# twndus/YelpRecommendation

Hardware: AMD Instinct MI355X
Metric: BPR triplets/sec @ dim64 (higher is better)
Workload: dtype f32; 1 GPU; BPR-MF dim=64 train step (gather+score+loss+grad+dense Adam), synthetic Yelp2018 shape; users=31668, items=38048, interactions=1566260, train_triplets_per_epoch=920629, batch_per_gpu=524288, global_batch=524288, optimizer=adam(dense), parallelism=single

## Files before the change

include/yelprec_engine.h:

```cpp
#ifndef YELPREC_ENGINE_H
#define YELPREC_ENGINE_H

#include <stdint.h>

#ifdef __cplusplus
extern "C" {
#endif

#define YR_ENGINE_VERSION 36

#define YR_ERR_UNSUPPORTED (-1)
#define YR_ERR_BADARG      (-2)

#define YR_FLAG_BAD_USER 1
#define YR_FLAG_BAD_ITEM 2

#define YR_PULL_USER_PHASE 1
#define YR_PULL_ITEM_PHASE 2

#define YR_S3REC_TRAIN 0
#define YR_S3REC_VALID 1
#define YR_S3REC_TEST  2

#define YR_OPT_ADAM  0
#define YR_OPT_ADAMW 1

#define YR_LOSS_PARTIALS 2048
#define YR_COUNT_SLOTS 64
#define YR_COUNT_WORDS 2048

int yr_engine_version(void);

const char *yr_engine_arch(void);

int yr_mf_score(const float *U, const float *I,
                const int64_t *user, const int64_t *item,
                int64_t B, int D, int64_t num_users, int64_t num_items,
                float *out, int32_t *err_flag, void *stream);

int yr_mf_score_backward(const float *U, const float *I,
                         const int64_t *user, const int64_t *item, const float *gout,
                         int64_t B, int D, int64_t num_users, int64_t num_items,
                         float *gradU, float *gradI, int32_t *err_flag, void *stream);

int yr_bpr_mf_fwd_bwd(const float *U, const float *I,
                      const int64_t *user, const int64_t *pos, const int64_t *neg,
                      int64_t B, int D, int64_t num_users, int64_t num_items,
                      float inv_batch, float *gradU, float *gradI,
                      float *loss_partials, int32_t *err_flag, void *stream);

int yr_bpr_mf_scatter_step(float *U, float *I, float *gradU, float *gradI,
                           float *mU, float *vU, float *mI, float *vI, uint8_t *touched,
                           const int64_t *user, const int64_t *pos, const int64_t *neg,
                           int64_t B, int D, int64_t num_users, int64_t num_items, float inv_batch,
                           double lr, double step_size, double bc2_sqrt,
                           double beta1, double beta2, double eps, double weight_decay, int mode,
                           float *loss_partials, float *loss_out, double *loss_accum,
                           int32_t *err_flag, void *stream);
int yr_adam_dense_dual(float *p0, float *g0, float *m0, float *v0, int64_t n0,
                       float *p1, float *g1, float *m1, float *v1, int64_t n1,
                       int row_width, uint8_t *touched0, uint8_t *touched1,
                       double lr, double step_size, double bc2_sqrt,
                       double beta1, double beta2, double eps, double weight_decay, int mode,
                       const float *loss_partials, float loss_scale, float *loss_out, double *loss_accum,
                       void *stream);

int64_t yr_bpr_mf_pull_workspace_bytes(int64_t max_batch, int64_t num_users, int64_t num_items, int D);
int yr_bpr_mf_pull_step(const float *U_old, float *U_new, float *I,
                        float *mU, float *vU, float *mI, float *vI, float *gradI_out,
                        const int64_t *user, const int64_t *pos, const int64_t *neg,
                        int64_t B, int D, int64_t num_users, int64_t num_items, float inv_batch,
                        double lr, double step_size, double bc2_sqrt,
                        double beta1, double beta2, double eps, double weight_decay, int mode,
                        int deterministic, void *workspace, int64_t workspace_bytes,
                        float *loss_partials, float *loss_out, double *loss_accum,
                        int32_t *err_flag, void *stream);

int yr_bpr_mf_pull_index(const int64_t *user, const int64_t *pos, const int64_t *neg, int64_t B, int D,
                         int64_t num_users, int64_t num_items,
                         void *workspace, int64_t workspace_bytes, int32_t *err_flag, void *stream);
int yr_bpr_mf_pull_apply(const float *U_old, float *U_new, float *I,
                         float *mU, float *vU, float *mI, float *vI, float *gradI_out,
                         int64_t B, int D, int64_t num_users, int64_t num_items, float inv_batch,
                         double lr, double step_size, double bc2_sqrt,
                         double beta1, double beta2, double eps, double weight_decay, int mode,
                         int deterministic, void *workspace, int64_t workspace_bytes,
                         float *loss_partials, float *loss_out, double *loss_accum,
                         int phases, int64_t item_row_begin, int64_t item_row_end,
                         void *stream);
int yr_bpr_mf_pull_item_buckets(int64_t num_items, int D);
int yr_bpr_mf_pull_split_summary(const void *workspace, int64_t workspace_bytes, int64_t B, int D,
                                 int64_t num_users, int64_t num_items, int32_t *counters_out,
                                 int32_t *parts_out, int32_t *rule_out, void *stream);
int yr_bpr_mf_pull_apply_ordered(const float *U_old, float *U_new, float *I,
                         float *mU, float *vU, float *mI, float *vI, float *gradI_out,
                         int64_t B, int D, int64_t num_users, int64_t num_items, float inv_batch,
                         double lr, double step_size, double bc2_sqrt,
                         double beta1, double beta2, double eps, double weight_decay, int mode,
                         int deterministic, void *workspace, int64_t workspace_bytes,
                         float *loss_partials, float *loss_out, double *loss_accum,
                         int phases, int64_t item_row_begin, int64_t item_row_end,
                         const int32_t *item_bucket_order, void *stream);

#define YR_NGCF_MAX_LAYERS 8
int yr_ngcf_score_fwd(const float *const *layers, int n_layers, const int64_t *user, const int64_t *pos,
                      const int64_t *neg, int64_t B, int D, int64_t num_users, int64_t num_items,
                      float *out_pos, float *out_neg, int32_t *err_flag, void *stream);
int yr_ngcf_score_bwd(const float *const *layers, float *const *dlayers, int n_layers, const int64_t *user,
                      const int64_t *pos, const int64_t *neg, const float *gpos, const float *gneg,
                      int64_t B, int D, int64_t num_users, int64_t num_items, int32_t *err_flag, void *stream);
int yr_spmm_csr(const int32_t *rowptr, const int32_t *col, const float *val,
                const float *X, float *Y, int64_t n, int D, int accumulate,
                const int32_t *heavy_rows, int64_t n_heavy, int heavy_threshold, void *stream);
int yr_spmm_csr_sliced(const int32_t *rowptr, const int32_t *col, const float *val,
                       const float *X, float *Y, int64_t n, int D, int accumulate,
                       const int32_t *row_order, void *stream);
int yr_ngcf_dense_fwd(const float *E, const float *Z, const float *W1, const float *W2,
                      int64_t n, int D, float *Eout, void *stream);
int yr_ngcf_dense_bwd_data(const float *dEout, const float *Eout, const float *E, const float *Z,
                           const float *W1T, const float *W2T, int64_t n, int D,
                           float *dZ, float *dE, void *stream);
int yr_ngcf_dense_bwd_weight(const float *dEout, const float *Eout, const float *E, const float *Z,
                             int64_t n, int D, float *dW1, float *dW2, void *stream);

int yr_ngcf_frontier_mark(const int64_t *user, const int64_t *pos, const int64_t *neg, int64_t B,
                          int64_t num_users, int64_t num_items,
                          int32_t *flags, int32_t *rows, int32_t *count, int clear, void *stream);
int yr_ngcf_frontier_expand(const int32_t *rowptr, const int32_t *col, int64_t n,
                            const int32_t *rows_in, const int32_t *count_in, int64_t max_rows_in,
                            int32_t *flags, int32_t *rows, int32_t *count, int clear, void *stream);
int yr_spmm_csr_subset(const int32_t *rowptr, const int32_t *col, const float *val,
                       const float *X, float *Y, int64_t n, int D, int accumulate,
                       const int32_t *heavy_rows, int64_t n_heavy, int heavy_threshold,
                       const int32_t *row_active,
                       const int32_t *row_list, const int32_t *row_count, int64_t max_rows, void *stream);
int yr_spmm_csr_push_rows(const int32_t *rowptr, const int32_t *col, const float *val,
                          const float *X, float *Y, int64_t n, int D,
                          const int32_t *rows, const int32_t *count, int64_t max_rows, void *stream);
int yr_ngcf_dense_fwd_rows(const float *E, const float *Z, const float *W1, const float *W2,
                           int64_t n, int D, float *Eout,
                           const int32_t *rows, const int32_t *count, int64_t max_rows, float *zero_rows,
                           void *stream);
int yr_ngcf_dense_bwd_data_rows(const float *dEout, const float *Eout, const float *E, const float *Z,
                                const float *W1T, const float *W2T, int64_t n, int D, float *dZ, float *dE,
                                const int32_t *rows, const int32_t *count, int64_t max_rows, void *stream);
int yr_ngcf_dense_bwd_weight_rows(const float *dEout, const float *Eout, const float *E, const float *Z,
                                  int64_t n, int D, float *dW1, float *dW2,
                                  const int32_t *rows, const int32_t *count, int64_t max_rows, void *stream);

int64_t yr_ngcf_step_workspace_bytes(int64_t n, int D, int K, int64_t B);
int yr_ngcf_bpr_step(const int32_t *rowptr, const int32_t *col, const float *val, int64_t n, int64_t nnz,
                     const int32_t *heavy_rows, int64_t n_heavy, int heavy_threshold, int64_t num_users,
                     float *const *params, float *const *exp_avg, float *const *exp_avg_sq, int K, int D,
                     const int64_t *user, const int64_t *pos, const int64_t *neg, int64_t B,
                     double lr, double step_size, double bc2_sqrt, double beta1, double beta2, double eps,
                     double weight_decay, int mode, double subset_fraction,
                     void *workspace, int64_t workspace_bytes, float *loss_out, double *loss_accum,
                     int32_t *err_flag, void *stream);

int yr_gemm_f32(int transA, int transB, int64_t M, int64_t N, int64_t K,
                const float *A, int64_t lda, const float *B, int64_t ldb, float *C, int64_t ldc,
                const float *bias, int act, int accumulate, int split_k, void *stream);
int yr_gemm_f32_ex(int transA, int transB, int64_t M, int64_t N, int64_t K,
                   const float *A, int64_t lda, const float *B, int64_t ldb, float *C, int64_t ldc,
                   const float *bias, int act, int accumulate, int split_k,
                   const int32_t *alpha_count, float *rowsum, void *stream);
int64_t yr_cdae_decode_loss_partials(int64_t B, int64_t I);
int yr_cdae_decode_loss(const float *z, const float *Wo, const float *bo, const float *target,
                        const float *negative_mask, int64_t B, int64_t I, int H, int act, float *G,
                        int64_t ldg, float *pred, float *partial_loss, int32_t *count, void *stream);
int yr_cdae_hidden_bwd(float *dz, const float *z, int act, const int64_t *user, int64_t B, int H,
                       int64_t num_users, float *dV, uint8_t *touched_users, float *dbh,
                       const float *partial_loss, int64_t n_partials, const int32_t *count,
                       float *stats, double *loss_accum, int scale_dz, void *stream);
int yr_cdae_compact_pair(const float *x, const float *negative_mask, int64_t B, int64_t I, uint64_t seed,
                         double p, int32_t *cols, float *vals, int32_t *count, int32_t *loss_cols,
                         float *loss_targets, int32_t *loss_count, void *stream);
int yr_cdae_train_lists(const int64_t *ptr, const int64_t *idx, const int64_t *ptr2, const int64_t *idx2,
                        const int64_t *users, int64_t B,
                        int64_t num_users, int64_t I, int neg_times, uint64_t neg_seed,
                        uint64_t drop_seed, double p, int32_t *cols, float *vals, int32_t *count,
                        int32_t *loss_cols, float *loss_targets, int32_t *loss_count,
                        int32_t *err_flag, void *stream);
int yr_cdae_train_lists_batched(const int64_t *ptr, const int64_t *idx, const int64_t *ptr2, const int64_t *idx2,
                                const int64_t *users, int64_t B, int64_t num_users, int64_t I, int neg_times,
                                const uint64_t *neg_seeds, const uint64_t *drop_seeds, int64_t batch_rows, double p,
                                int32_t *cols, float *vals, int32_t *count, int32_t *loss_cols, float *loss_targets,
                                int32_t *loss_count, int32_t *err_flag, void *stream);
int yr_cdae_loss_finalize_batched(const float *partial_loss, int splits, const int32_t *loss_count, int64_t rows,
                                  int64_t batch_rows, float *means, int32_t *arrive, double *loss_accum,
                                  void *stream);
int yr_cdae_sampled_decode_splits(int64_t B);
int yr_cdae_loss_finalize(const float *partial_loss, int64_t n_partials, const int32_t *count, float *stats,
                          double *loss_accum, void *stream);
int yr_cdae_sampled_decode(const int32_t *loss_cols, const float *loss_targets, const int32_t *loss_count,
                           const float *z, const float *Wo, const float *bo, int64_t B, int64_t I, int H,
                           int act, float *dz, float *dWo, float *dbo, float *partial_loss,
                           int32_t *count, void *stream);
int yr_cdae_hidden_init(float *zpre, const float *bias, const float *V, const int64_t *user,
                        int64_t B, int H, int64_t num_users, int32_t *err_flag, void *stream);
int yr_dropout(const float *x, const float *rnd, double p, int64_t n, float *out, void *stream);
int yr_sigmoid(float *x, int64_t n, void *stream);
int yr_dropout_seeded(const float *x, uint64_t seed, double p, int64_t n, float *out, void *stream);
int yr_sigmoid_bwd(const float *dy, const float *y, float *g, int64_t n, void *stream);
int yr_colsum(const float *X, int64_t rows, int64_t cols, float *out, int accumulate, void *stream);
int yr_row_scatter_add(const float *G, const int64_t *user, int64_t B, int H, int64_t num_users,
                       float *dV, void *stream);
int yr_nsbce_fwd(const float *pred, const float *target, const float *negative_mask, int64_t n,
                 float *workspace, float *stats, void *stream);
int yr_nsbce_bwd(const float *pred, const float *target, const float *negative_mask,
                 const float *stats, const float *gout, int64_t n, float *dpred, void *stream);

int yr_loss_finalize(const float *loss_partials, float scale,
                     float *loss_out, double *loss_accum, void *stream);

int yr_mf_scores_gemm(const float *U, const float *I, const int64_t *users, int64_t nrows, int D,
                      int64_t num_users, int64_t num_items, float *scores, int64_t row_stride,
                      int32_t *err_flag, void *stream);

#define YR_EVAL_F32 0
#define YR_EVAL_BF16X3 1
#define YR_EVAL_NO_PRESCAN 2
#define YR_EVAL_FORCE_PRESCAN 4
#define YR_EVAL_TWO_ROLES 8
#define YR_EVAL_FOUR_WAVES 16
int64_t yr_mf_eval_topk_planes_bytes(int64_t num_items, int D);
int64_t yr_mf_eval_topk_workspace_bytes(int64_t nrows, int64_t num_items, int D, int k, int mode);
int yr_mf_eval_topk(const float *U, const float *I, const int64_t *users, int64_t nrows, int D,
                    int64_t num_users, int64_t num_items,
                    const int64_t *mask_ptr, const int64_t *mask_idx, float mask_value,
                    int k, int64_t *out, void *workspace, int64_t workspace_bytes, int mode,
                    const int64_t *hint, int32_t *err_flag, void *stream);
int yr_mf_eval_topk_bias(const float *U, const float *I, const float *item_bias, const int64_t *users,
                         int64_t nrows, int D, int64_t num_users, int64_t num_items,
                         const int64_t *mask_ptr, const int64_t *mask_idx, float mask_value,
                         int k, int64_t *out, void *workspace, int64_t workspace_bytes, int mode,
                         const int64_t *hint, int32_t *err_flag, void *stream);
int64_t yr_ngcf_eval_topk_workspace_bytes(int64_t nrows, int64_t num_items, int n_layers, int D, int k);
int yr_ngcf_eval_topk(const float *const *layers, int n_layers, int D, const int64_t *users, int64_t nrows,
                      int64_t num_users, int64_t num_items,
                      const int64_t *mask_ptr, const int64_t *mask_idx, float mask_value,
                      int k, int64_t *out, void *workspace, int64_t workspace_bytes,
                      const int64_t *hint, int32_t *err_flag, void *stream);

int yr_topk_masked(const float *scores, int64_t nrows, int64_t ncols, int64_t row_stride,
                   const int64_t *mask_ptr, const int64_t *mask_idx, const int64_t *mask_rows,
                   float mask_value, int k, int64_t *out, void *stream);

int64_t yr_rank_metrics_workspace_bytes(int64_t n);
int yr_rank_metrics(const int64_t *topk, int64_t n, int k, const int64_t *pos_ptr, const int64_t *pos_idx,
                    const int64_t *pos_rows, double *workspace, double *out, void *stream);

int yr_bpr_loss_fwd(const float *pos, const float *neg, int64_t B,
                    float *loss_partials, void *stream);
int yr_bpr_loss_bwd(const float *pos, const float *neg, const float *gout,
                    float inv_batch, int64_t B, float *gpos, float *gneg, void *stream);

int yr_adam_dense(float *p, float *g, float *m, float *v, int64_t n,
                  double lr, double step_size, double bc2_sqrt,
                  double beta1, double beta2, double eps, double weight_decay,
                  int mode, int zero_grad, void *stream);

#define YR_ADAM_MULTI_MAX 16
int yr_adam_dense_flat(float *const *p, float *const *g, float *const *m, float *const *v,
                       const int64_t *n, uint8_t *const *touched, const int *row_width, const int *clear,
                       const int *scaled, const int32_t *grad_count, int count, double lr, double step_size, double bc2_sqrt, double beta1,
                       double beta2, double eps, double weight_decay, int mode, void *stream);
int yr_sgd_dense(float *p, float *g, int64_t n, double lr, double weight_decay,
                 int zero_grad, void *stream);

int yr_csr_rows_to_dense(const int64_t *ptr, const int64_t *idx, const int64_t *users, int64_t B,
                         int64_t num_users, int64_t num_items, int accumulate, float *out,
                         int32_t *err_flag, void *stream);
int yr_negative_mask(const float *positives, int64_t B, int64_t num_items, int neg_times, uint64_t seed,
                     float *out, int32_t *err_flag, void *stream);

int64_t yr_cdae_sparse_part_columns(int64_t I);
int yr_cdae_compact_rows(const float *x, int64_t B, int64_t I, uint64_t seed, double p,
                         int32_t *cols, float *vals, int32_t *count, void *stream);
int yr_cdae_sparse_encode(const int32_t *cols, const float *vals, const int32_t *count,
                          const float *Wh, const float *bh, const float *V, const int64_t *user,
                          int64_t B, int64_t I, int H, int64_t num_users, int act, float *z,
                          int32_t *err_flag, void *stream);
int yr_cdae_sparse_dwh(const int32_t *cols, const float *vals, const int32_t *count,
                       const float *dz, int64_t B, int64_t I, int H, float *dWh,
                       float *scratch_T, int32_t *claim, int32_t epoch, int32_t *touched, int32_t *n_touched,
                       void *stream);
int yr_cdae_sparse_encode_t(const int32_t *cols, const float *vals, const int32_t *count, const float *WhT,
                            const float *bh, const float *V, const int64_t *user, int64_t B, int64_t I,
                            int H, int64_t num_users, int act, float *z, int32_t *err_flag, void *stream);
int yr_cdae_sparse_dwh_t(const int32_t *cols, const float *vals, const int32_t *count, const float *dz,
                         int64_t B, int64_t I, int H, float *dWhT, uint8_t *touched_items, void *stream);
int yr_cdae_hidden_bwd_dwh_t(const int32_t *cols, const float *vals, const int32_t *count, const float *dz,
                             const float *z, int act, int scale_dz, const int32_t *pos_count,
                             const int64_t *user, int64_t B, int64_t I, int H, int64_t num_users, float *dV,
                             uint8_t *touched_users, float *dbh, float *dWhT, uint8_t *touched_items,
                             const float *partial_loss, int64_t n_partials, float *stats,
                             double *loss_accum, void *stream);

int64_t yr_cdae_catalogue_bce_workspace_floats(int64_t B, int64_t I, int H);
int yr_cdae_catalogue_bce(const float *z, const float *Wo, const float *bo, const int64_t *user,
                          const int64_t *tgt_ptr, const int64_t *tgt_idx, int64_t B, int64_t I, int64_t K, int H,
                          int act, float *row_loss, float *dz, float *dWo, float *dbo, float *workspace,
                          int64_t workspace_floats, int32_t *err_flag, void *stream);

int yr_triplet_sample(const int64_t *row_user, const int64_t *row_item, int64_t n_rows,
                      const int64_t *avoid_ptr, const int64_t *avoid_idx,
                      int64_t num_users, int64_t num_items, uint64_t seed, uint64_t epoch, int shuffle,
                      int64_t first, int64_t count,
                      int64_t *user_out, int64_t *pos_out, int64_t *neg_out,
                      int32_t *err_flag, void *stream);

int yr_dcn_assemble(const float *U, const float *I, const float *C, const float *S, const int32_t *cat_ids,
                    const int32_t *sc_ids, int Lmax, int D, int64_t num_users, int64_t num_items, int64_t num_cats,
                    int64_t num_sc, const int64_t *user, const int64_t *item_a, const int64_t *item_b, int64_t B,
                    int attr_per_row, float *x, int64_t ldx, int32_t *err_flag, void *stream);
int yr_dcn_assemble_bwd(const float *dx, int64_t ldx, const int32_t *cat_ids, const int32_t *sc_ids, int Lmax, int D,
                        int64_t num_users, int64_t num_items, int64_t num_cats, int64_t num_sc, const int64_t *user,
                        const int64_t *item_a, const int64_t *item_b, int64_t B, int attr_per_row, float *gU,
                        float *gI, float *gC, float *gS, int32_t *err_flag, void *stream);
int yr_relu_bwd(float *g, const float *y, int64_t n, void *stream);
int yr_dcn_head(const float *x0, int64_t ldx, const float *h, int64_t ldh, int64_t units, int F, int H, int L,
                const float *cw, const float *cb, const float *Wo, const float *bo, int bpr, float inv_batch,
                float *pred, const float *gpred, float *dh, int64_t lddh, float *dx0, int64_t lddx, float *dcw,
                float *dcb, float *dWo, float *dbo, float *loss_partials, void *stream);
int yr_dcn_score(const float *Au, int64_t ldau, const float *Bi, int64_t ldbi, const float *Pu, const float *Pi,
                 const int64_t *users, int64_t n_eval, int64_t num_users, int64_t num_items, int H1, int H2,
                 const float *W2, const float *b2, const float *Wo, const float *bo, const float *cw, const float *cb,
                 int L, int F, float *scores, int64_t row_stride, int32_t *err_flag, void *stream);

int yr_s3rec_encode(const float *item_emb, const float *pos_enc, const float *params, const int64_t *X, int64_t B,
                    int L, int E, int heads, int blocks, int64_t num_items, int last_only, float *out,
                    int32_t *err_flag, void *stream);
int yr_s3rec_seq_scores(const float *item_emb, const float *h, const int64_t *pos_items, const int64_t *neg_items,
                        int64_t rows, int E, int64_t num_items, float *pos_preds, float *neg_preds,
                        int32_t *err_flag, void *stream);
int yr_s3rec_candidate_scores(const float *item_emb, const float *h_last, const int64_t *pos_item,
                              const int64_t *neg_items, int64_t B, int64_t C, int E, int64_t num_items,
                              float *pos_pred, float *neg_preds, int32_t *err_flag, void *stream);

int64_t yr_s3rec_train_workspace_floats(int64_t B, int L, int E, int heads, int blocks);
int yr_s3rec_encode_train(const float *item_emb, const float *pos_enc, const float *params, const int64_t *X,
                          int64_t B, int L, int E, int heads, int blocks, int64_t num_items, uint64_t seed, double p,
                          float *out, float *workspace, int64_t workspace_floats, int32_t *err_flag, void *stream);
int yr_s3rec_backward(const float *params, const int64_t *X, const float *dh_out, int64_t B, int L, int E, int heads,
                      int blocks, uint64_t seed, double p, float *workspace, int64_t workspace_floats, float *d_emb,
                      void *stream);
int yr_s3rec_score_grad(const float *item_emb, const int64_t *pos_items, const int64_t *neg_items,
                        const float *dpos_preds, const float *dneg_preds, int64_t rows, int E, int64_t num_items,
                        float *dh_out, int32_t *err_flag, void *stream);
int yr_s3rec_item_grad(const int64_t *sorted_ids, const int64_t *order, const float *d_emb, const float *h,
                       const float *dpos_preds, const float *dneg_preds, int64_t rows, int E, int64_t num_items,
                       float *partial, float *d_item, int32_t *err_flag, void *stream);

int64_t yr_s3rec_catalogue_bce_workspace_floats(int64_t N, int64_t R, int E);
int yr_s3rec_catalogue_bce(const float *F, const float *T, const float *zscale, const float *yscale,
                           const int64_t *key, const int64_t *tgt_ptr, const int64_t *tgt_idx, int64_t N, int64_t R,
                           int64_t K, int E, float *loss, float *row_loss, float *dF, float *dT, float *workspace,
                           int64_t workspace_floats, int32_t *err_flag, void *stream);

int64_t yr_s3rec_catalogue_rank_workspace_bytes(int64_t N, int64_t R, int E);
int yr_s3rec_catalogue_rank(const float *H, const float *T, const int64_t *target, const int64_t *excl_ptr,
                            const int64_t *excl_idx, const int64_t *excl_rows, int64_t N, int64_t R, int64_t K, int E,
                            int64_t first_col, int64_t *rank, float *target_score, void *workspace,
                            int64_t workspace_bytes, int32_t *err_flag, void *stream);

int yr_s3rec_batches(const int64_t *beh_ptr, const int64_t *beh_idx, const int64_t *avoid_ptr,
                     const int64_t *avoid_idx, int64_t num_users, int64_t num_items, const int64_t *users, int64_t B,
                     int L, int mode, int n_neg, uint64_t seed, uint64_t epoch, int64_t *X, int64_t *pos,
                     int64_t *neg, int32_t *err_flag, void *stream);

#ifdef __cplusplus
}
#endif
#endif
```

yelprecommendation_amd/_lib.py:

```python
from __future__ import annotations

import ctypes as C
import os

_HERE = os.path.dirname(os.path.abspath(__file__))
LIB_PATH = os.environ.get("YR_ENGINE_LIB") or os.path.join(_HERE, "libyelprec_engine.so")
ENGINE_VERSION = 36

_p = C.c_void_p
_i64 = C.c_int64
_int = C.c_int
_f = C.c_float
_d = C.c_double

SIGNATURES = {
    "yr_engine_version": [],
    "yr_engine_arch": [],
    "yr_mf_score": [_p, _p, _p, _p, _i64, _int, _i64, _i64, _p, _p, _p],
    "yr_mf_score_backward": [_p, _p, _p, _p, _p, _i64, _int, _i64, _i64, _p, _p, _p, _p],
    "yr_bpr_mf_fwd_bwd": [_p, _p, _p, _p, _p, _i64, _int, _i64, _i64, _f, _p, _p, _p, _p, _p],
    "yr_bpr_mf_scatter_step": [_p, _p, _p, _p, _p, _p, _p, _p, _p, _p, _p, _p, _i64, _int, _i64, _i64, _f,
                               _d, _d, _d, _d, _d, _d, _d, _int, _p, _p, _p, _p, _p],
    "yr_adam_dense_dual": [_p, _p, _p, _p, _i64, _p, _p, _p, _p, _i64, _int, _p, _p,
                           _d, _d, _d, _d, _d, _d, _d, _int, _p, _f, _p, _p, _p],
    "yr_bpr_mf_pull_workspace_bytes": [_i64, _i64, _i64, _int],
    "yr_bpr_mf_pull_step": [_p, _p, _p, _p, _p, _p, _p, _p, _p, _p, _p, _i64, _int, _i64, _i64, _f,
                            _d, _d, _d, _d, _d, _d, _d, _int, _int, _p, _i64, _p, _p, _p, _p, _p],
    "yr_spmm_csr": [_p, _p, _p, _p, _p, _i64, _int, _int, _p, _i64, _int, _p],
    "yr_spmm_csr_sliced": [_p, _p, _p, _p, _p, _i64, _int, _int, _p, _p],
    "yr_ngcf_score_fwd": [_p, _int, _p, _p, _p, _i64, _int, _i64, _i64, _p, _p, _p, _p],
    "yr_ngcf_score_bwd": [_p, _p, _int, _p, _p, _p, _p, _p, _i64, _int, _i64, _i64, _p, _p],
    "yr_ngcf_dense_fwd": [_p, _p, _p, _p, _i64, _int, _p, _p],
    "yr_ngcf_dense_bwd_data": [_p, _p, _p, _p, _p, _p, _i64, _int, _p, _p, _p],
    "yr_ngcf_dense_bwd_weight": [_p, _p, _p, _p, _i64, _int, _p, _p, _p],
    "yr_ngcf_frontier_mark": [_p, _p, _p, _i64, _i64, _i64, _p, _p, _p, _int, _p],
    "yr_ngcf_frontier_expand": [_p, _p, _i64, _p, _p, _i64, _p, _p, _p, _int, _p],
    "yr_spmm_csr_subset": [_p, _p, _p, _p, _p, _i64, _int, _int, _p, _i64, _int, _p, _p, _p, _i64, _p],
    "yr_spmm_csr_push_rows": [_p, _p, _p, _p, _p, _i64, _int, _p, _p, _i64, _p],
    "yr_ngcf_dense_fwd_rows": [_p, _p, _p, _p, _i64, _int, _p, _p, _p, _i64, _p, _p],
    "yr_ngcf_dense_bwd_data_rows": [_p, _p, _p, _p, _p, _p, _i64, _int, _p, _p, _p, _p, _i64, _p],
    "yr_ngcf_dense_bwd_weight_rows": [_p, _p, _p, _p, _i64, _int, _p, _p, _p, _p, _i64, _p],
    "yr_ngcf_step_workspace_bytes": [_i64, _int, _int, _i64],
    "yr_ngcf_bpr_step": [_p, _p, _p, _i64, _i64, _p, _i64, _int, _i64, _p, _p, _p, _int, _int, _p, _p, _p, _i64,
                         _d, _d, _d, _d, _d, _d, _d, _int, _d, _p, _i64, _p, _p, _p, _p],
    "yr_gemm_f32": [_int, _int, _i64, _i64, _i64, _p, _i64, _p, _i64, _p, _i64, _p, _int, _int, _int, _p],
    "yr_gemm_f32_ex": [_int, _int, _i64, _i64, _i64, _p, _i64, _p, _i64, _p, _i64, _p, _int, _int, _int, _p, _p, _p],
    "yr_cdae_decode_loss_partials": [_i64, _i64],
    "yr_cdae_decode_loss": [_p, _p, _p, _p, _p, _i64, _i64, _int, _int, _p, _i64, _p, _p, _p, _p],
    "yr_cdae_hidden_bwd": [_p, _p, _int, _p, _i64, _int, _i64, _p, _p, _p, _p, _i64, _p, _p, _p, _int, _p],
    "yr_cdae_compact_pair": [_p, _p, _i64, _i64, C.c_uint64, _d, _p, _p, _p, _p, _p, _p, _p],
    "yr_cdae_train_lists": [_p, _p, _p, _p, _p, _i64, _i64, _i64, _int, C.c_uint64, C.c_uint64, _d, _p, _p, _p, _p, _p,
                            _p, _p, _p],
    "yr_cdae_train_lists_batched": [_p, _p, _p, _p, _p, _i64, _i64, _i64, _int, _p, _p, _i64, _d, _p, _p, _p, _p, _p,
                                    _p, _p, _p],
    "yr_cdae_loss_finalize_batched": [_p, _int, _p, _i64, _i64, _p, _p, _p, _p],
    "yr_cdae_loss_finalize": [_p, _i64, _p, _p, _p, _p],
    "yr_cdae_sampled_decode_splits": [_i64],
    "yr_cdae_sampled_decode": [_p, _p, _p, _p, _p, _p, _i64, _i64, _int, _int, _p, _p, _p, _p, _p, _p],
    "yr_cdae_hidden_init": [_p, _p, _p, _p, _i64, _int, _i64, _p, _p],
    "yr_dropout": [_p, _p, _d, _i64, _p, _p],
    "yr_sigmoid": [_p, _i64, _p],
    "yr_dropout_seeded": [_p, C.c_uint64, _d, _i64, _p, _p],
    "yr_sigmoid_bwd": [_p, _p, _p, _i64, _p],
    "yr_colsum": [_p, _i64, _i64, _p, _int, _p],
    "yr_row_scatter_add": [_p, _p, _i64, _int, _i64, _p, _p],
    "yr_nsbce_fwd": [_p, _p, _p, _i64, _p, _p, _p],
    "yr_nsbce_bwd": [_p, _p, _p, _p, _p, _i64, _p, _p],
    "yr_bpr_mf_pull_index": [_p, _p, _p, _i64, _int, _i64, _i64, _p, _i64, _p, _p],
    "yr_bpr_mf_pull_apply": [_p, _p, _p, _p, _p, _p, _p, _p, _i64, _int, _i64, _i64, _f,
                             _d, _d, _d, _d, _d, _d, _d, _int, _int, _p, _i64, _p, _p, _p, _int, _i64, _i64, _p],
    "yr_bpr_mf_pull_apply_ordered": [_p, _p, _p, _p, _p, _p, _p, _p, _i64, _int, _i64, _i64, _f,
                             _d, _d, _d, _d, _d, _d, _d, _int, _int, _p, _i64, _p, _p, _p, _int, _i64, _i64, _p, _p],
    "yr_bpr_mf_pull_item_buckets": [_i64, _int],
    "yr_bpr_mf_pull_split_summary": [_p, _i64, _i64, _int, _i64, _i64, _p, _p, _p, _p],
    "yr_loss_finalize": [_p, _f, _p, _p, _p],
    "yr_mf_scores_gemm": [_p, _p, _p, _i64, _int, _i64, _i64, _p, _i64, _p, _p],
    "yr_mf_eval_topk_planes_bytes": [_i64, _int],
    "yr_mf_eval_topk_workspace_bytes": [_i64, _i64, _int, _int, _int],
    "yr_mf_eval_topk": [_p, _p, _p, _i64, _int, _i64, _i64, _p, _p, _f, _int, _p, _p, _i64, _int, _p, _p, _p],
    "yr_mf_eval_topk_bias": [_p, _p, _p, _p, _i64, _int, _i64, _i64, _p, _p, _f, _int, _p, _p, _i64, _int, _p, _p, _p],
    "yr_ngcf_eval_topk_workspace_bytes": [_i64, _i64, _int, _int, _int],
    "yr_ngcf_eval_topk": [_p, _int, _int, _p, _i64, _i64, _i64, _p, _p, _f, _int, _p, _p, _i64, _p, _p, _p],
    "yr_topk_masked": [_p, _i64, _i64, _i64, _p, _p, _p, _f, _int, _p, _p],
    "yr_rank_metrics_workspace_bytes": [_i64],
    "yr_rank_metrics": [_p, _i64, _int, _p, _p, _p, _p, _p, _p],
    "yr_bpr_loss_fwd": [_p, _p, _i64, _p, _p],
    "yr_bpr_loss_bwd": [_p, _p, _p, _f, _i64, _p, _p, _p],
    "yr_adam_dense": [_p, _p, _p, _p, _i64, _d, _d, _d, _d, _d, _d, _d, _int, _int, _p],
    "yr_adam_dense_flat": [_p, _p, _p, _p, _p, _p, _p, _p, _p, _p, _int, _d, _d, _d, _d, _d, _d, _d, _int, _p],
    "yr_csr_rows_to_dense": [_p, _p, _p, _i64, _i64, _i64, _int, _p, _p, _p],
    "yr_negative_mask": [_p, _i64, _i64, _int, C.c_uint64, _p, _p, _p],
    "yr_sgd_dense": [_p, _p, _i64, _d, _d, _int, _p],
    "yr_cdae_sparse_part_columns": [_i64],
    "yr_cdae_compact_rows": [_p, _i64, _i64, C.c_uint64, _d, _p, _p, _p, _p],
    "yr_cdae_sparse_encode": [_p, _p, _p, _p, _p, _p, _p, _i64, _i64, _int, _i64, _int, _p, _p, _p],
    "yr_cdae_sparse_dwh": [_p, _p, _p, _p, _i64, _i64, _int, _p, _p, _p, C.c_int32, _p, _p, _p],
    "yr_cdae_sparse_encode_t": [_p, _p, _p, _p, _p, _p, _p, _i64, _i64, _int, _i64, _int, _p, _p, _p],
    "yr_cdae_sparse_dwh_t": [_p, _p, _p, _p, _i64, _i64, _int, _p, _p, _p],
    "yr_cdae_hidden_bwd_dwh_t": [_p, _p, _p, _p, _p, _int, _int, _p, _p, _i64, _i64, _int, _i64, _p, _p, _p, _p, _p, _p,
                                 _i64, _p, _p, _p],
    "yr_cdae_catalogue_bce_workspace_floats": [_i64, _i64, _int],
    "yr_cdae_catalogue_bce": [_p, _p, _p, _p, _p, _p, _i64, _i64, _i64, _int, _int, _p, _p, _p, _p, _p, _i64, _p, _p],
    "yr_triplet_sample": [_p, _p, _i64, _p, _p, _i64, _i64, C.c_uint64, C.c_uint64, _int, _i64, _i64,
                          _p, _p, _p, _p, _p],
    "yr_dcn_assemble": [_p, _p, _p, _p, _p, _p, _int, _int, _i64, _i64, _i64, _i64, _p, _p, _p, _i64, _int, _p, _i64,
                        _p, _p],
    "yr_dcn_assemble_bwd": [_p, _i64, _p, _p, _int, _int, _i64, _i64, _i64, _i64, _p, _p, _p, _i64, _int, _p, _p, _p,
                            _p, _p, _p],
    "yr_relu_bwd": [_p, _p, _i64, _p],
    "yr_dcn_head": [_p, _i64, _p, _i64, _i64, _int, _int, _int, _p, _p, _p, _p, _int, _f, _p, _p, _p, _i64, _p, _i64,
                    _p, _p, _p, _p, _p, _p],
    "yr_dcn_score": [_p, _i64, _p, _i64, _p, _p, _p, _i64, _i64, _i64, _int, _int, _p, _p, _p, _p, _p, _p, _int, _int,
                     _p, _i64, _p, _p],
    "yr_s3rec_encode": [_p, _p, _p, _p, _i64, _int, _int, _int, _int, _i64, _int, _p, _p, _p],
    "yr_s3rec_seq_scores": [_p, _p, _p, _p, _i64, _int, _i64, _p, _p, _p, _p],
    "yr_s3rec_candidate_scores": [_p, _p, _p, _p, _i64, _i64, _int, _i64, _p, _p, _p, _p],
    "yr_s3rec_train_workspace_floats": [_i64, _int, _int, _int, _int],
    "yr_s3rec_encode_train": [_p, _p, _p, _p, _i64, _int, _int, _int, _int, _i64, C.c_uint64, _d, _p, _p, _i64, _p, _p],
    "yr_s3rec_backward": [_p, _p, _p, _i64, _int, _int, _int, _int, C.c_uint64, _d, _p, _i64, _p, _p],
    "yr_s3rec_score_grad": [_p, _p, _p, _p, _p, _i64, _int, _i64, _p, _p, _p],
    "yr_s3rec_item_grad": [_p, _p, _p, _p, _p, _p, _i64, _int, _i64, _p, _p, _p, _p],
    "yr_s3rec_catalogue_bce_workspace_floats": [_i64, _i64, _int],
    "yr_s3rec_catalogue_bce": [_p, _p, _p, _p, _p, _p, _p, _i64, _i64, _i64, _int, _p, _p, _p, _p, _p, _i64, _p, _p],
    "yr_s3rec_catalogue_rank_workspace_bytes": [_i64, _i64, _int],
    "yr_s3rec_catalogue_rank": [_p, _p, _p, _p, _p, _p, _i64, _i64, _i64, _int, _i64, _p, _p, _p, _i64, _p, _p],
    "yr_s3rec_batches": [_p, _p, _p, _p, _i64, _i64, _p, _i64, _int, _int, _int, C.c_uint64, C.c_uint64, _p, _p, _p, _p,
                         _p],
}

RESTYPES = {"yr_engine_arch": C.c_char_p}
RESTYPES.update({name: _i64 for name in (
    "yr_bpr_mf_pull_workspace_bytes", "yr_rank_metrics_workspace_bytes", "yr_cdae_sparse_part_columns",
    "yr_cdae_decode_loss_partials", "yr_mf_eval_topk_workspace_bytes", "yr_mf_eval_topk_planes_bytes",
    "yr_ngcf_step_workspace_bytes", "yr_ngcf_eval_topk_workspace_bytes", "yr_s3rec_train_workspace_floats",
    "yr_s3rec_catalogue_bce_workspace_floats", "yr_s3rec_catalogue_rank_workspace_bytes",
    "yr_cdae_catalogue_bce_workspace_floats")})

_lib = None


class EngineError(RuntimeError):
    pass


def load():
    global _lib
    if _lib is not None:
        return _lib
    import torch
    if not os.path.exists(LIB_PATH):
        raise EngineError(
            f"HIP engine library not found at {LIB_PATH}. Build it with "
            "`python -c 'import __graft_entry__ as g; g.build()'` or "
            "`make -C yelprecommendation_amd/csrc`. There is no CPU/PyTorch fallback.")
    try:
        lib = C.CDLL(LIB_PATH)
    except OSError as e:
        raise EngineError(f"cannot load {LIB_PATH}: {e}") from e
    for name, argtypes in SIGNATURES.items():
        try:
            fn = getattr(lib, name)
        except AttributeError as e:
            raise EngineError(f"{LIB_PATH} does not export {name}") from e
        fn.argtypes = argtypes
        fn.restype = RESTYPES.get(name, C.c_int)
    v = lib.yr_engine_version()
    if v != ENGINE_VERSION:
        raise EngineError(f"engine ABI version {v} != expected {ENGINE_VERSION}; rebuild the library")
    _lib = lib
    return lib


def check(status: int, what: str):
    if status == 0:
        return
    if status == -1:
        raise EngineError(f"{what}: unsupported configuration (embedding width must be 16/32/64/128, or 256/512/1024 on the BPR-MF push, evaluation and score paths; top-k above 16 needs a width up to 64)")
    if status == -2:
        raise EngineError(f"{what}: bad argument (null pointer, negative size or misaligned buffer)")
    raise EngineError(f"{what}: HIP error {status}")
```

yelprecommendation_amd/bpr_step.py:

```python
import torch

from . import engine
from .user_shard import ItemSlices, reduce_scatter_item_exchange, sharded_item_exchange


AUTO_PULL_MIN_BATCH = 24576

IMPL_NAMES = {
    "auto": "auto: atomic scatter + one Adam launch below %d triplets per rank and step, pull above" % AUTO_PULL_MIN_BATCH,
    "pull": "pull: tile partition + owner pass per table (gather/score/loss/grad/Adam fused, no atomics)",
    "atomic": "atomic: fused gather/score/loss + float-atomic scatter-add, dense Adam",
}


class BPRMFStep:
    def __init__(self, U, I, lr=1e-4, betas=(0.9, 0.999), eps=1e-8, weight_decay=0.0, optimizer="adam",
                 world_size=1, process_group=None, time_kernels=False, impl="auto", max_batch=0,
                 state=None, split_item_update=False, item_chunks=1, item_exchange="all_reduce", rank=0,
                 deterministic=False):
        if item_exchange not in ("all_reduce", "reduce_scatter"):
            raise ValueError("item_exchange must be 'all_reduce' or 'reduce_scatter'")
        width = int(U.shape[1])
        if width in engine.WIDE_WIDTHS:
            limit = max(engine.SUPPORTED_WIDTHS)
            for wanted, what in ((impl == "pull", 'impl="pull"'), (bool(deterministic), "deterministic=True"),
                                 (item_exchange == "reduce_scatter", 'item_exchange="reduce_scatter"')):
                if wanted:
                    raise NotImplementedError(
                        f"BPRMFStep: {what} needs the pull form, which covers embedding widths up to {limit}; "
                        f"width {width} trains with the push form only (impl=\"auto\" or \"atomic\")")
        self.deterministic = bool(deterministic)
        self.skip_collective = False
        self.item_exchange = item_exchange
        self.rank = int(rank)
        self.split_item_update = split_item_update
        self.item_chunks = max(1, int(item_chunks))
        if optimizer.lower() not in ("adam", "adamw"):
            raise NotImplementedError(f"BPRMFStep: optimizer {optimizer}")
        if impl not in IMPL_NAMES:
            raise ValueError(f"impl must be one of {list(IMPL_NAMES)}")
        self.impl_key, self.impl = impl, IMPL_NAMES[impl]
        self.launches = ""
        self.U, self.I = U, I
        self._U_alt = None
        self._ws_slots, self._ws_batch, self._indexed = [None, None], [0, 0], None
        if impl == "pull" and max_batch:
            self._workspace(max_batch, 0)
        self._gI_dirty = False
        self._touched = None
        self._item_order, self.auto_item_order = None, True
        self.lr, self.betas, self.eps, self.wd = lr, betas, eps, weight_decay
        self.decoupled = optimizer.lower() == "adamw"
        self.world_size, self.pg = world_size, process_group
        dev = U.device
        self.gU = None
        self.gI = torch.zeros_like(I) if (world_size > 1 or split_item_update) else None
        self._slices = self._I_pad = None
        if item_exchange == "reduce_scatter" and (world_size > 1 or split_item_update):
            self._slices = ItemSlices(I.shape[0], world_size, self.rank)
            self._gI_pad = torch.zeros(self._slices.padded, I.shape[1], dtype=I.dtype, device=I.device)
            self.gI = self._gI_pad[:I.shape[0]]
            self._I_pad = torch.zeros(self._slices.padded, I.shape[1], dtype=I.dtype, device=I.device)
        if state is not None:
            self.mU, self.vU, self.mI, self.vI = state["mU"], state["vU"], state["mI"], state["vI"]
            self.t = int(state.get("t", 0))
        else:
            self.mU, self.vU = torch.zeros_like(U), torch.zeros_like(U)
            self.mI, self.vI = torch.zeros_like(I), torch.zeros_like(I)
            self.t = 0
        self.partials = torch.zeros(engine.LOSS_PARTIALS, dtype=torch.float32, device=dev)
        self.loss = torch.zeros(1, dtype=torch.float32, device=dev)
        self.loss_accum = torch.zeros(1, dtype=torch.float64, device=dev)
        self.flag = engine.new_error_flag(dev)
        self.time_kernels = time_kernels
        self._ev = {}
        self._bytes = {}
        from . import _lib
        self._lib = _lib.load()
        f32 = torch.float32
        for name, t in (("U", U), ("I", I), ("mU", self.mU), ("vU", self.vU), ("mI", self.mI), ("vI", self.vI)):
            engine._dev(t, f32, name)
        if U.dim() != 2 or I.dim() != 2 or U.shape[1] != I.shape[1]:
            raise engine.EngineError("tables must be [rows, D] with equal D")
        if self.mU.shape != U.shape or self.vU.shape != U.shape or self.mI.shape != I.shape or self.vI.shape != I.shape:
            raise engine.EngineError("Adam state must match the table shapes")
        self._pI, self._pmU, self._pvU = I.data_ptr(), self.mU.data_ptr(), self.vU.data_ptr()
        self._pmI, self._pvI = self.mI.data_ptr(), self.vI.data_ptr()
        self._ppartials, self._pflag = self.partials.data_ptr(), self.flag.data_ptr()
        self._pull_ok = self._lib.yr_bpr_mf_pull_workspace_bytes(1, U.shape[0], I.shape[0], U.shape[1]) > 0 and \
            engine.pull_supported(U.shape[0], I.shape[0], U.shape[1])

    def reset_timers(self):
        self._ev = {}

    def _timed(self, name, alg_bytes, record, fn):
        if not (record and self.time_kernels):
            return fn()
        a, b = torch.cuda.Event(enable_timing=True), torch.cuda.Event(enable_timing=True)
        a.record()
        fn()
        b.record()
        self._ev.setdefault(name, []).append((a, b))
        self._bytes[name] = alg_bytes

    def kernel_times(self):
        torch.cuda.synchronize()
        return {k: (sum(a.elapsed_time(b) for a, b in v) * 1e3 / len(v), len(v), self._bytes[k])
                for k, v in self._ev.items()}

    def _workspace(self, batch, slot=0):
        ws = self._ws_slots[slot]
        if ws is None or batch > self._ws_batch[slot]:
            ws = engine.bpr_mf_pull_workspace(batch, self.U.shape[0], self.I.shape[0], self.U.shape[1],
                                              self.U.device)
            self._ws_slots[slot], self._ws_batch[slot] = ws, batch
        return ws

    def step(self, u, p, n, record=False, global_batch=None, next_batch=None):
        if global_batch is None:
            global_batch = u.numel() * self.world_size
        key = self.impl_key
        if key == "auto":
            key = "pull" if (global_batch >= AUTO_PULL_MIN_BATCH * self.world_size and self._pull_ok) else "atomic"
            if self._slices is not None or self.deterministic:
                key = "pull"
        if key == "pull":
            if self._U_alt is None:
                self._U_alt = torch.empty_like(self.U)
            self.impl = IMPL_NAMES["pull"]
            self.launches = "tile_partition, owner_pass<user>, owner_pass<item>"
            return self._step_pull(u, p, n, record, global_batch, next_batch)
        if self.gU is None:
            self.gU = torch.zeros_like(self.U)
        if self.gI is None:
            self.gI = torch.zeros_like(self.I)
        self.impl = IMPL_NAMES["atomic"]
        self.launches = "bpr_fwd_bwd, adam_dual"
        return self._step_atomic(u, p, n, record, global_batch)

    def _check_triplets(self, u, p, n):
        B = u.numel()
        for name, t in (("user", u), ("pos", p), ("neg", n)):
            if not (t.is_cuda and t.dtype == torch.int64 and t.is_contiguous() and t.numel() == B):
                raise engine.EngineError(f"{name}: need a contiguous int64 GPU tensor of length {B}")
        return B

    def _build_index(self, u, p, n, slot):
        B = self._check_triplets(u, p, n)
        ws = self._workspace(B, slot)
        rc = self._lib.yr_bpr_mf_pull_index(u.data_ptr(), p.data_ptr(), n.data_ptr(), B, self.U.shape[1],
                                            self.U.shape[0], self.I.shape[0], ws.data_ptr(), ws.numel(),
                                            self._pflag, engine._stream())
        if rc:
            engine.check(rc, "yr_bpr_mf_pull_index")
        self._indexed = (slot, (u, p, n))

    def set_item_order(self, item_weight=None):
        if item_weight is None:
            self._item_order = None
            return
        nb = int(self._lib.yr_bpr_mf_pull_item_buckets(self.I.shape[0], self.I.shape[1]))
        rows = -(-self.I.shape[0] // nb) if nb else 1
        per = 1024 // self.I.shape[1]
        w = torch.zeros(nb * per, dtype=torch.float64, device=self.I.device)
        w[:self.I.shape[0]] = item_weight.to(self.I.device, torch.float64)
        load = w.view(nb, per).sum(1)
        self._item_order = torch.argsort(load, descending=True, stable=True).to(torch.int32).contiguous()

    def _auto_item_order(self, p, n):
        rows = self.I.shape[0]
        ids = torch.cat([p, n])
        ids = ids[(ids >= 0) & (ids < rows)]
        self.set_item_order(torch.bincount(ids, minlength=rows)[:rows])

    def _step_pull(self, u, p, n, record, global_batch, next_batch=None):
        B = u.numel()
        D = self.U.shape[1]
        if self._item_order is None and self.auto_item_order and B >= 4 * self.I.shape[0]:
            self._auto_item_order(p, n)
        inv = 1.0 / global_batch if global_batch else 0.0
        self.t += 1
        multi = self.world_size > 1 or self.split_item_update
        nU, nI = self.U.numel(), self.I.numel()
        alg = B * (24 + 24 * D) + 6 * 4 * (nU + (0 if multi else nI))
        ready = self._indexed is not None and all(a is b for a, b in zip(self._indexed[1], (u, p, n)))
        slot = self._indexed[0] if ready else 0

        nchunks = self.item_chunks if multi else 1
        rows = self.I.shape[0]
        gran = engine.pull_bucket_rows(D)
        bounds = [min(rows, (rows * c // nchunks + gran - 1) // gran * gran) for c in range(nchunks)] + [rows]
        both = engine.PULL_USER_PHASE | engine.PULL_ITEM_PHASE
        ploss, paccum = self.loss.data_ptr(), self.loss_accum.data_ptr()

        def apply(phases, r0, r1, with_loss=None):
            ws = self._ws_slots[slot]
            if with_loss is None:
                with_loss = bool(phases & engine.PULL_USER_PHASE)
            step_size, bc2_sqrt = engine.adam_scalars(self.t, self.lr, self.betas[0], self.betas[1])
            order = self._item_order
            rc = self._lib.yr_bpr_mf_pull_apply_ordered(
                self.U.data_ptr(), self._U_alt.data_ptr(), self._pI, self._pmU, self._pvU, self._pmI, self._pvI,
                self.gI.data_ptr() if multi else None, B, D, self.U.shape[0], rows, inv, self.lr,
                step_size, bc2_sqrt, self.betas[0], self.betas[1], self.eps, self.wd,
                engine.OPT_ADAMW if self.decoupled else engine.OPT_ADAM, 1 if self.deterministic else 0,
                ws.data_ptr(), ws.numel(), self._ppartials, ploss if with_loss else None,
                paccum if with_loss else None, phases, r0, r1, order.data_ptr() if order is not None else None,
                engine._stream())
            if rc:
                engine.check(rc, "yr_bpr_mf_pull_apply_ordered")

        def first_chunk():
            if not ready:
                self._build_index(u, p, n, slot)
            apply(both, bounds[0], bounds[1])
            if nchunks == 1:
                self._indexed = None

        def local_first():
            if record and self.time_kernels and not multi and self.t % 2 == 0:
                self._timed("tile_partition", B * 24, record,
                            lambda: None if ready else self._build_index(u, p, n, slot))
                self._timed("owner_pass_user", B * (16 * D), record,
                            lambda: apply(engine.PULL_USER_PHASE, 0, 0, with_loss=False))
                self._timed("owner_pass_item", B * (8 * D), record,
                            lambda: apply(engine.PULL_ITEM_PHASE, bounds[0], bounds[1], with_loss=True))
                self._indexed = None
                return
            self._timed("bpr_pull_step", alg, record, first_chunk)

        def make_chunk(c):
            def run():
                apply(engine.PULL_ITEM_PHASE, bounds[c], bounds[c + 1])
                if c == nchunks - 1:
                    self._indexed = None
            return run

        def overlap():
            if next_batch is not None:
                self._build_index(*next_batch, 1 - slot)

        def make_update(c):
            def run():
                if multi:
                    r0, r1 = bounds[c], bounds[c + 1]
                    self._timed("adam_dense_item", 7 * 4 * (r1 - r0) * D, record, lambda: engine.adam_dense(
                        self.I[r0:r1], self.gI[r0:r1], self.mI[r0:r1], self.vI[r0:r1], self.t, self.lr,
                        self.betas[0], self.betas[1], self.eps, self.wd, decoupled=self.decoupled, zero_grad=False))
            return run

        if multi and self._slices is not None:
            sl = self._slices

            def whole_item_pass():
                local_first()
                for c in range(1, nchunks):
                    make_chunk(c)()

            def slice_update():
                lo, hi, at = sl.lo, sl.hi, sl.rank * sl.per
                if hi > lo:
                    self._timed("adam_dense_item_slice", 7 * 4 * (hi - lo) * D, record, lambda: engine.adam_dense(
                        self.I[lo:hi], self._gI_pad[at:at + hi - lo], self.mI[lo:hi], self.vI[lo:hi], self.t, self.lr,
                        self.betas[0], self.betas[1], self.eps, self.wd, decoupled=self.decoupled, zero_grad=False))
                    self._I_pad[at:at + hi - lo].copy_(self.I[lo:hi])

            reduce_scatter_item_exchange(whole_item_pass, slice_update, self._gI_pad, self._I_pad, sl, self.pg, overlap,
                                         collective=not self.skip_collective)
            if self.world_size > 1 and not self.skip_collective:
                self.I.copy_(self._I_pad[:rows])
            self._gI_dirty = True
            self.U, self._U_alt = self._U_alt, self.U
            return
        steps = [local_first] + [make_chunk(c) for c in range(1, nchunks)]
        grads = [self.gI[bounds[c]:bounds[c + 1]] for c in range(nchunks)] if multi else [None]
        sharded_item_exchange(steps, [make_update(c) for c in range(nchunks)], grads, self.pg, self.world_size,
                              overlap, collective=not self.skip_collective)
        self._gI_dirty = multi
        self.U, self._U_alt = self._U_alt, self.U

    def _step_atomic(self, u, p, n, record, global_batch):
        B = self._check_triplets(u, p, n)
        D = self.U.shape[1]
        inv = 1.0 / global_batch if global_batch else 0.0
        lib, stream = self._lib, engine._stream()
        if self._gI_dirty:
            self.gI.zero_()
            self._gI_dirty = False
        nU, nI = self.U.shape[0], self.I.shape[0]
        pU, pgU, pgI = self.U.data_ptr(), self.gU.data_ptr(), self.gI.data_ptr()
        self.t += 1
        step_size, bc2_sqrt = engine.adam_scalars(self.t, self.lr, self.betas[0], self.betas[1])
        mode = engine.OPT_ADAMW if self.decoupled else engine.OPT_ADAM
        ploss, paccum = self.loss.data_ptr(), self.loss_accum.data_ptr()
        if self.world_size == 1:
            if self._touched is None:
                self._touched = torch.zeros(nU + nI, dtype=torch.uint8, device=self.U.device)

            def whole():
                rc = lib.yr_bpr_mf_scatter_step(pU, self._pI, pgU, pgI, self._pmU, self._pvU, self._pmI, self._pvI,
                                                self._touched.data_ptr(), u.data_ptr(), p.data_ptr(), n.data_ptr(),
                                                B, D, nU, nI, inv, self.lr, step_size, bc2_sqrt, self.betas[0],
                                                self.betas[1], self.eps, self.wd, mode, self._ppartials, ploss,
                                                paccum, self._pflag, stream)
                if rc:
                    engine.check(rc, "yr_bpr_mf_scatter_step")

            self._timed("bpr_scatter_step", B * (24 + 24 * D) + 6 * 4 * (nU + nI) * D, record, whole)
            return

        def fwd_bwd():
            rc = lib.yr_bpr_mf_fwd_bwd(pU, self._pI, u.data_ptr(), p.data_ptr(), n.data_ptr(), B, D, nU, nI, inv,
                                       pgU, pgI, self._ppartials, self._pflag, stream)
            if rc:
                engine.check(rc, "yr_bpr_mf_fwd_bwd")

        self._timed("bpr_fwd_bwd", B * (24 + 24 * D), record, fwd_bwd)
        if not self.skip_collective:
            import torch.distributed as dist
            dist.all_reduce(self.gI, op=dist.ReduceOp.SUM, group=self.pg)

        def adam():
            rc = lib.yr_adam_dense_dual(pU, pgU, self._pmU, self._pvU, nU * D, self._pI, pgI, self._pmI, self._pvI,
                                        nI * D, D, None, None, self.lr, step_size, bc2_sqrt, self.betas[0],
                                        self.betas[1], self.eps, self.wd, mode, self._ppartials, inv, ploss, paccum,
                                        stream)
            if rc:
                engine.check(rc, "yr_adam_dense_dual")

        self._timed("adam_dense_dual", 8 * 4 * (nU + nI) * D, record, adam)

    def epoch_loss(self, reset=True):
        if self.world_size > 1:
            import torch.distributed as dist
            dist.all_reduce(self.loss_accum, op=dist.ReduceOp.SUM, group=self.pg)
        v = float(self.loss_accum.item())
        if reset:
            self.loss_accum.zero_()
        return v

    def check(self):
        engine.raise_on_flag(self.flag, "BPRMFStep")
```

yelprecommendation_amd/csrc/bpr_pull.hip:

```cpp
#include "adam.h"
#include "common.h"

namespace yr {

constexpr int kPartThreads = 1024;
#ifndef YR_ITEM_CAP
#define YR_ITEM_CAP 1024
#endif
constexpr int kCap = YR_ITEM_CAP;
constexpr int kUserCap = 768;
constexpr int kTileGroup = 256;
constexpr int kOccShift = 26;
constexpr int kOccMask = (1 << kOccShift) - 1;
constexpr int kMaxBuckets = 16383;
constexpr int kMaxOwnerGrid = 4096;
#ifndef YR_HEAVY_ROW
#define YR_HEAVY_ROW 96
#endif
constexpr int kHeavyRow = YR_HEAVY_ROW;
#ifndef YR_SPLIT_MIN
#define YR_SPLIT_MIN 2048
#endif
constexpr int kSplitMin = YR_SPLIT_MIN;
#ifndef YR_SPLIT_AVG_MIN
#define YR_SPLIT_AVG_MIN 2.5
#endif
#ifndef YR_SPLIT_AVG_TARGET
#define YR_SPLIT_AVG_TARGET 1.25
#endif
#ifndef YR_SPLIT_TARGET
#define YR_SPLIT_TARGET 1024
#endif
constexpr int kSplitTarget = YR_SPLIT_TARGET;
constexpr int kMaxParts = 64;
constexpr int kMaxTasks = 512;
constexpr int kMaxSlots = 1024;
#ifndef YR_ROWSPLIT
#define YR_ROWSPLIT 1
#endif
#ifndef YR_ROWSPLIT_MIN
#define YR_ROWSPLIT_MIN 1024
#endif
#ifndef YR_ROWSPLIT_AVG_MIN
#define YR_ROWSPLIT_AVG_MIN 2.32
#endif
#ifndef YR_ROWSPLIT_TARGET
#define YR_ROWSPLIT_TARGET 512
#endif
#ifndef YR_ROWSPLIT_AVG_TARGET
#define YR_ROWSPLIT_AVG_TARGET 1.16
#endif
constexpr int kRowSplitMin = YR_ROWSPLIT_MIN;
constexpr int kRowSplitTarget = YR_ROWSPLIT_TARGET;
constexpr int kMaxRowTasks = YR_ROWSPLIT ? 512 : 0;
constexpr int kBuildLanes = 4;
#ifndef YR_DEAL
#define YR_DEAL 1
#endif
#ifndef YR_DEAL_MIN
#define YR_DEAL_MIN 256
#endif
constexpr int kDealMin = YR_DEAL_MIN;
#ifndef YR_OWNER_WAVES
#define YR_OWNER_WAVES 8
#endif
#ifndef YR_USER_UNROLL
#define YR_USER_UNROLL 1
#endif
#ifndef YR_ITEM_UNROLL
#define YR_ITEM_UNROLL 2
#endif
constexpr int kUserUnroll = YR_USER_UNROLL;
constexpr int kItemUnroll = YR_ITEM_UNROLL;

struct PullAdam {
  AdamScalars c;
  int decoupled;
};

__device__ __forceinline__ float4 ld4o(const float* base, uint32_t off) {
  return *reinterpret_cast<const float4*>(reinterpret_cast<const char*>(base) + (uint32_t)(off * 4u));
}

template <int D>
struct PullGeom {
  static_assert(D == 16 || D == 32 || D == 64 || D == 128, "unsupported width");
  static constexpr int LPR = D / 4;
  static constexpr int GPW = kWave / LPR;
  static constexpr int R = kWavesPerBlock * GPW;
};
#ifndef YR_MIN_TILES
#define YR_MIN_TILES 64
#endif
constexpr int kMinTiles = YR_MIN_TILES;
constexpr int kNarrowRows = kWavesPerBlock;
constexpr int kNarrowShift = 2;
#ifndef YR_NARROW_BELOW
#define YR_NARROW_BELOW 768
#endif
constexpr int kNarrowBelow = YR_NARROW_BELOW;

inline int bucket_shift(int D) { return D == 16 ? 6 : D == 32 ? 5 : D == 64 ? 4 : 3; }

template <int PT>
__global__ __launch_bounds__(kPartThreads) void tile_partition_kernel(
    const int64_t* __restrict__ user, const int64_t* __restrict__ pos, const int64_t* __restrict__ neg, int64_t B,
    int64_t nU, int64_t nI, int shiftU, int shiftI, int nbU, int nbI, int32_t* __restrict__ offU,
    int32_t* __restrict__ offI,
    int4* __restrict__ rec, int2* __restrict__ occ, int32_t* __restrict__ err_flag, int stage_off,
    int32_t* __restrict__ split_counters) {
  extern __shared__ int32_t s_cnt[];
  __shared__ int s_wave[kPartThreads / kWave];
  int4* s_stage = reinterpret_cast<int4*>(s_cnt + stage_off);
  constexpr int TILE = kPartThreads * PT;
  const int side = blockIdx.y, tile = blockIdx.x, tid = threadIdx.x;
  if (side == 0 && tile == 0) {
    if (tid < 3) split_counters[tid] = 0;
    for (int i = tid; i < nbI; i += kPartThreads) split_counters[4 + i] = 1;
  }
  const int nb = side ? nbI : nbU;
  const int shift = side ? shiftI : shiftU;
  const int rmask = (1 << shift) - 1;

  int32_t u[PT], p[PT], n[PT];
  int bad = 0;
#pragma unroll
  for (int k = 0; k < PT; ++k) {
    const int64_t b = (int64_t)tile * TILE + (int64_t)k * kPartThreads + tid;
    u[k] = -1; p[k] = 0; n[k] = 0;
    if (b < B) {
      const int64_t uu = user[b], pp = pos[b], nn = neg[b];
      int f = 0;
      if ((uint64_t)uu >= (uint64_t)nU) f |= YR_FLAG_BAD_USER;
      if ((uint64_t)pp >= (uint64_t)nI || (uint64_t)nn >= (uint64_t)nI) f |= YR_FLAG_BAD_ITEM;
      if (f) bad |= f;
      else { u[k] = (int32_t)uu; p[k] = (int32_t)pp; n[k] = (int32_t)nn; }
    }
  }
  for (int i = tid; i <= nb; i += kPartThreads) s_cnt[i] = 0;
  __syncthreads();
  int ra[PT], rb[PT];
#pragma unroll
  for (int k = 0; k < PT; ++k) {
    ra[k] = 0; rb[k] = 0;
    if (u[k] >= 0) {
      if (side == 0) {
        ra[k] = atomicAdd(&s_cnt[u[k] >> shift], 1);
      } else {
        ra[k] = atomicAdd(&s_cnt[p[k] >> shift], 1);
        rb[k] = atomicAdd(&s_cnt[n[k] >> shift], 1);
      }
    }
  }
  __syncthreads();
  {
    const int per = (nb + kPartThreads - 1) / kPartThreads;
    const int i0 = tid * per;
    int sum = 0;
    for (int i = i0; i < i0 + per && i < nb; ++i) sum += s_cnt[i];
    const int lane = tid & (kWave - 1), wave = tid / kWave;
    int inc = sum;
#pragma unroll
    for (int d = 1; d < kWave; d <<= 1) {
      const int o = __shfl_up(inc, d, kWave);
      if (lane >= d) inc += o;
    }
    if (lane == kWave - 1) s_wave[wave] = inc;
    __syncthreads();
    int before = inc - sum;
    for (int w = 0; w < wave; ++w) before += s_wave[w];
    for (int i = i0; i < i0 + per && i < nb; ++i) {
      const int c = s_cnt[i];
      s_cnt[i] = before;
      before += c;
    }
    if (tid == kPartThreads - 1) s_cnt[nb] = before;
  }
  __syncthreads();
  int32_t* off = (side ? offI : offU) + (int64_t)tile * (nb + 1);
  for (int i = tid; i <= nb; i += kPartThreads) off[i] = s_cnt[i];
  const int total = s_cnt[nb];
  if (side == 0) {
#pragma unroll
    for (int k = 0; k < PT; ++k)
      if (u[k] >= 0) {
        const int b = tile * TILE + k * kPartThreads + tid;
        s_stage[s_cnt[u[k] >> shift] + ra[k]] = make_int4(p[k], n[k], b, u[k] & rmask);
      }
    if (bad && err_flag) atomicOr(err_flag, bad);
    __syncthreads();
    int4* out = rec + (int64_t)tile * TILE;
    for (int i = tid; i < total; i += kPartThreads) out[i] = s_stage[i];
  } else {
    int2* stage2 = reinterpret_cast<int2*>(s_stage);
#pragma unroll
    for (int k = 0; k < PT; ++k)
      if (u[k] >= 0) {
        const int b = tile * TILE + k * kPartThreads + tid;
        stage2[s_cnt[p[k] >> shift] + ra[k]] = make_int2(u[k] | ((p[k] & rmask) << kOccShift), b);
        stage2[s_cnt[n[k] >> shift] + rb[k]] = make_int2(u[k] | ((n[k] & rmask) << kOccShift), b | (int)0x80000000);
      }
    __syncthreads();
    int4* out = reinterpret_cast<int4*>(occ + (int64_t)tile * TILE * 2);
    const int n16 = (total + 1) >> 1;
    for (int i = tid; i < n16; i += kPartThreads) out[i] = s_stage[i];
  }
}

#ifdef YR_STAMPS
__device__ long long g_stamps[8192 * 8];
__device__ int g_walk_iters[8192 * 4];
#define YR_STAMP(i) do { if (threadIdx.x == 0 && first_bucket) g_stamps[(blockIdx.x + (USER ? 0 : 4096)) * 8 + (i)] = wall_clock64(); } while (0)
#else
#define YR_STAMP(i)
#endif

struct OwnerArgs {
  const float* own_old;
  float* own_new;
  const float* other;
  float* m;
  float* v;
  float* grad_out;
  const int32_t* off;
  const void* recs;
  float* coeff;
  float* loss_partials;
  float* loss_out;
  double* loss_accum;
  int finalize;
  int nb, T, tile_stride;
  int rows;
  int bucket_begin, bucket_end;
  const int32_t* order;
  int heavy_t;
  float inv_batch;
  PullAdam adam;
  char* split;
  float* scratch;
  const int32_t* b_off;
  int helper_blocks, build_blocks, b_nb;
  int b_split_min, b_split_target;
  int b_rowsplit_min, b_rowsplit_quad;
};

__host__ __device__ __forceinline__ size_t split_per(int nbI) { return ((size_t)nbI * 4 + 15) & ~(size_t)15; }
__device__ __forceinline__ int32_t* split_counters(char* b) { return (int32_t*)b; }
__device__ __forceinline__ int32_t* split_parts(char* b) { return (int32_t*)(b + 16); }
__device__ __forceinline__ int32_t* split_slot(char* b, int nbI) { return (int32_t*)(b + 16 + split_per(nbI)); }
__device__ __forceinline__ int32_t* split_arrive(char* b, int nbI) { return (int32_t*)(b + 16 + 2 * split_per(nbI)); }
__device__ __forceinline__ int4* split_tasks(char* b, int nbI) { return (int4*)(b + 16 + 3 * split_per(nbI)); }
__device__ __forceinline__ int2* split_row_tasks(char* b, int nbI) { return (int2*)(split_tasks(b, nbI) + kMaxTasks); }

__device__ __forceinline__ void build_splits(const OwnerArgs& a, int builder) {
  const int k = (builder * kBlock + (int)threadIdx.x) / kBuildLanes, j = threadIdx.x % kBuildLanes;
  int total = 0;
  if (k < a.b_nb) {
    int t = j;
    const int64_t pitch = a.b_nb + 1;
    for (; t + 3 * kBuildLanes < a.T; t += 4 * kBuildLanes) {
      const int32_t* o0 = a.b_off + (int64_t)t * pitch + k;
      const int32_t* o1 = o0 + kBuildLanes * pitch;
      const int32_t* o2 = o1 + kBuildLanes * pitch;
      const int32_t* o3 = o2 + kBuildLanes * pitch;
      const int a0 = o0[0], b0 = o0[1], a1 = o1[0], b1 = o1[1], a2 = o2[0], b2 = o2[1], a3 = o3[0], b3 = o3[1];
      total += ((b0 - a0) + (b1 - a1)) + ((b2 - a2) + (b3 - a3));
    }
    for (; t < a.T; t += kBuildLanes) {
      const int32_t* orow = a.b_off + (int64_t)t * (a.b_nb + 1) + k;
      total += orow[1] - orow[0];
    }
  }
#pragma unroll
  for (int m = 1; m < kBuildLanes; m <<= 1) total += __shfl_xor(total, m, kWave);
  if (k >= a.b_nb || j != 0) return;
  int parts = 1;
  if (total >= a.b_split_min) {
    parts = (total + a.b_split_target - 1) / a.b_split_target;
    parts = min(parts, min(kMaxParts, a.T));
  }
  int slot = 0;
  if (parts > 1) {
    slot = atomicAdd(split_counters(a.split) + 1, parts);
    const int first = atomicAdd(split_counters(a.split), parts - 1);
    const bool fits = slot + parts <= kMaxSlots && first + parts - 1 <= kMaxTasks;
    for (int q = 1; q < parts; ++q)
      if (first + q - 1 < kMaxTasks) split_tasks(a.split, a.b_nb)[first + q - 1] = make_int4(fits ? k : -1, q, 0, 0);
    if (!fits) parts = 1;
  }
#if YR_ROWSPLIT
  else if (total < a.b_split_min && total >= a.b_rowsplit_min) {
    const int S = total >= a.b_rowsplit_quad ? 4 : 2;
    const int first = atomicAdd(split_counters(a.split) + 2, S - 1);
    for (int q = 1; q < S; ++q)
      if (first + q - 1 < kMaxRowTasks) split_row_tasks(a.split, a.b_nb)[first + q - 1] = make_int2(k, q);
    parts = -S;
  }
#endif
  split_parts(a.split)[k] = parts;
  split_slot(a.split, a.b_nb)[k] = slot;
  split_arrive(a.split, a.b_nb)[k] = 0;
}

template <int LPR>
__device__ __forceinline__ void cross_group_sum(float4& a) {
#pragma unroll
  for (int m = LPR; m < kWave; m <<= 1) {
    a.x += __shfl_xor(a.x, m, kWave);
    a.y += __shfl_xor(a.y, m, kWave);
    a.z += __shfl_xor(a.z, m, kWave);
    a.w += __shfl_xor(a.w, m, kWave);
  }
}

__device__ __forceinline__ int wave_inclusive_scan(int x, int lane) {
#pragma unroll
  for (int d = 1; d < kWave; d <<= 1) {
    const int t = __shfl_up(x, d, kWave);
    if (lane >= d) x += t;
  }
  return x;
}

template <int LPR, int GPW>
struct RowSums {
  float4 total;
  __device__ __forceinline__ void clear() { total = zero4(); }
  __device__ __forceinline__ void book(bool closing, int cur_row, const float4& cur, int grp) {
#pragma unroll 1
    for (int j = 0; j < GPW; ++j) {
      const bool sel = closing && cur_row == j;
      if (!__ballot(sel)) continue;
      float4 v = sel ? cur : zero4();
      cross_group_sum<LPR>(v);
      if (grp == j) { total.x += v.x; total.y += v.y; total.z += v.z; total.w += v.w; }
    }
  }
  __device__ __forceinline__ float4 finish(int) { return total; }
};

template <int R, int RPW>
__device__ __forceinline__ void deal_rows(const int* s_cnt, unsigned char* s_slotof, unsigned char* s_rowof, int lane,
                                          int heavy_t) {
  static_assert(kWavesPerBlock == 4 && R == 4 * RPW, "four waves of RPW slots");
  const int c = s_cnt[lane];
  const int load = (lane < R && c <= heavy_t) ? c : 0;
  const int order = (load << 6) | (kWave - 1 - lane);
  int rank = 0;
  for (int j = 0; j < R; ++j) rank += __builtin_amdgcn_readlane(order, j) > order ? 1 : 0;
  int wkey = lane < kWavesPerBlock ? lane : 0x7fffffff, wused = 0;
  int slot = lane;
  for (int i = 0; i < R; ++i) {
    const int src = __builtin_amdgcn_readfirstlane(__ffsll((unsigned long long)__ballot(lane < R && rank == i)) - 1);
    const int ci = __builtin_amdgcn_readlane(load, src);
    const int w = min(min(__builtin_amdgcn_readlane(wkey, 0), __builtin_amdgcn_readlane(wkey, 1)),
                      min(__builtin_amdgcn_readlane(wkey, 2), __builtin_amdgcn_readlane(wkey, 3))) & 3;
    const int s = w * RPW + __builtin_amdgcn_readlane(wused, w);
    if (lane == w) {
      wused += 1;
      wkey = wused == RPW ? 0x7fffffff : wkey + (ci << 2);
    }
    if (lane == src) slot = s;
  }
  s_slotof[lane] = (unsigned char)slot;
  s_rowof[slot] = (unsigned char)lane;
}

constexpr int kTagShift = 10;
constexpr int kTagMask = (1 << kTagShift) - 1;

template <int D, bool USER, bool HEAVY, bool LOOKUP>
__device__ __forceinline__ void walk_stream(const OwnerArgs& a, const unsigned short* s_idx, const int* s_x,
                                            const int* s_y, const int* s_z, const float4* s_own,
                                            const unsigned char* s_slotof, int lo, int hi,
                                            int first, int stride, int row_base, int grp, int l,
                                            RowSums<PullGeom<D>::LPR, PullGeom<D>::GPW>& sums, float4& cur,
                                            float& loss) {
  using G = PullGeom<D>;
  constexpr int LPR = G::LPR;
  constexpr int N = USER ? kUserUnroll : kItemUnroll;
  int cur_row = -1;
  for (int base = lo; base < hi; base += stride * N) {
    bool valid[N];
    int tag[N], ia[N], ib[N], ic[N];
    float4 r0[N], r1[N];
#pragma unroll
    for (int q = 0; q < N; ++q) {
      const int pos = base + first + q * stride;
      valid[q] = pos < hi;
      const int e = s_idx[min(pos, hi - 1)];
      tag[q] = e >> kTagShift;
      const int c = e & kTagMask;
      ia[q] = s_x[c];
      ib[q] = s_y[c];
      ic[q] = USER ? s_z[c] : 0;
    }
#pragma unroll
    for (int q = 0; q < N; ++q) {
      r0[q] = ld4o(a.other, (uint32_t)(ia[q] * D + 4 * l));
      if (USER) r1[q] = ld4o(a.other, (uint32_t)(ib[q] * D + 4 * l));
    }
#pragma unroll
    for (int q = 0; q < N; ++q) {
      if (!HEAVY) {
        const bool closing = valid[q] && cur_row >= 0 && tag[q] != cur_row;
        if (__ballot(closing)) {
          const int slot = LOOKUP ? (int)s_slotof[max(cur_row, 0)] : cur_row;
          sums.book(closing, slot - row_base, cur, grp);
          if (closing) cur = zero4();
        }
        if (valid[q]) cur_row = tag[q];
      }
      if (USER) {
        const float4 ownj = s_own[tag[q] * LPR + l];
        float4 d;
        d.x = r0[q].x - r1[q].x; d.y = r0[q].y - r1[q].y; d.z = r0[q].z - r1[q].z; d.w = r0[q].w - r1[q].w;
        float part = ownj.x * d.x;
        part = fmaf(ownj.y, d.y, part);
        part = fmaf(ownj.z, d.z, part);
        part = fmaf(ownj.w, d.w, part);
        const float x = group_sum_dpp<LPR>(part);
        float sp, sg;
        bpr_terms(x, sp, sg);
        const float gg = valid[q] ? -sg * a.inv_batch : 0.0f;
        cur.x = fmaf(gg, d.x, cur.x); cur.y = fmaf(gg, d.y, cur.y);
        cur.z = fmaf(gg, d.z, cur.z); cur.w = fmaf(gg, d.w, cur.w);
        if (valid[q] && l == 0) {
          a.coeff[ic[q]] = gg;
          loss += sp;
        }
      } else {
        const float gg = valid[q] ? __int_as_float(ib[q]) : 0.0f;
        cur.x = fmaf(gg, r0[q].x, cur.x); cur.y = fmaf(gg, r0[q].y, cur.y);
        cur.z = fmaf(gg, r0[q].z, cur.z); cur.w = fmaf(gg, r0[q].w, cur.w);
      }
    }
  }
  if (!HEAVY) {
    const int slot = LOOKUP ? (int)s_slotof[max(cur_row, 0)] : cur_row;
    sums.book(cur_row >= 0, slot - row_base, cur, grp);
  }
}

__device__ __forceinline__ bool row_kept(int row, int part, int parts) {
  return !YR_ROWSPLIT || ((row ^ part) & max(-parts - 1, 0)) == 0;
}

template <bool USER>
__device__ __forceinline__ int walk_steps(int n, int groups) {
  const int per = groups * (USER ? kUserUnroll : kItemUnroll);
  return (n + per - 1) / per;
}


template <int D_, bool USER_, bool FUSE_ADAM_, bool DET_, int RPWX>
struct OwnerForm {
  static constexpr int D = D_;
  static constexpr bool USER = USER_, FUSE_ADAM = FUSE_ADAM_, DET = DET_;
  static constexpr int LPR = PullGeom<D>::LPR, GPW = PullGeom<D>::GPW;
  static constexpr int RPW = RPWX ? RPWX : GPW;
  static_assert(RPW <= GPW, "a wave finishes at most one row per lane group");
  static constexpr int R = kWavesPerBlock * RPW;
  static constexpr int DEAL_BAR = kDealMin * (kWavesPerBlock * GPW) * (kWavesPerBlock * GPW) / 256;
  static constexpr bool DEAL = RPWX == 0 && YR_DEAL && DEAL_BAR <= (USER ? kUserCap : kCap);
  static constexpr bool TAG_SLOT = DEAL && !USER, LOOKUP = DEAL && USER;
  static constexpr int CAP = USER ? kUserCap : kCap;
  static constexpr int PT = CAP / kBlock;
};

struct OwnerLds {
  int *pre, *base, *cnt, *start;
  unsigned char* rowof;
  int *x, *y, *z;
  unsigned short* idx;
  int *scan, *n, *last;
};

__device__ __forceinline__ int tile_of(const int* s_pre, int nt, int j) {
  int tlo = 0, thi = nt;
  while (thi - tlo > 1) {
    const int mid = (tlo + thi) >> 1;
    if (s_pre[mid] <= j) tlo = mid; else thi = mid;
  }
  return tlo;
}

__device__ __forceinline__ int scan_segments(const OwnerArgs& a, const OwnerLds& s, int tid, int k, int tg0,
                                             int nt) {
  const int lane = tid & (kWave - 1), wave = tid / kWave;
  int len = 0;
  if (tid < nt) {
    const int32_t* orow = a.off + (int64_t)(tg0 + tid) * (a.nb + 1) + k;
    const int o0 = orow[0], o1 = orow[1];
    len = o1 - o0;
    s.base[tid] = (tg0 + tid) * a.tile_stride + o0;
  }
  int inc = 0, before = 0;
  if (nt > kWave) {
    inc = wave_inclusive_scan(len, lane);
    if (lane == kWave - 1) s.scan[wave] = inc;
    __syncthreads();
    for (int w = 0; w < wave; ++w) before += s.scan[w];
  } else if (wave == 0) {
    inc = wave_inclusive_scan(len, lane);
  }
  if (nt > kWave || wave == 0) {
    s.pre[tid] = before + inc - len;
    if (lane == kWave - 1) s.pre[tid + 1] = before + inc;
  }
  __syncthreads();
  return s.pre[nt];
}

template <int CAP>
__device__ __forceinline__ bool cut_chunk_at_tiles(const int* s_pre, int nt, int c0, int total, int& cend, int& wt) {
  wt = tile_of(s_pre, nt, c0);
  const bool windowed = s_pre[wt + 1] - s_pre[wt] > CAP;
  if (!windowed && cend < total) {
    const int tb = tile_of(s_pre, nt, cend);
    if (s_pre[tb] > c0) cend = s_pre[tb];
  }
  return windowed;
}

template <class F>
__device__ __forceinline__ int load_window(const OwnerArgs& a, const OwnerLds& s, int tid, int part,
                                           int parts, int tg0, int wt, int c0, int& sub, int& cend,
                                           int (&key)[F::PT]) {
  constexpr bool USER = F::USER;
  constexpr int CAP = F::CAP, PT = F::PT;
  constexpr int W = USER ? CAP : CAP / 2;
  const int tile_ids = USER ? a.tile_stride : a.tile_stride >> 1;
  const int seg = s.pre[wt + 1] - s.pre[wt];
  const uint32_t rbase = (uint32_t)s.base[wt];
  const uint32_t id_lo = (uint32_t)(tg0 + wt) * (uint32_t)tile_ids + (uint32_t)sub * (uint32_t)W;
  for (int sidx = tid; sidx < seg; sidx += kBlock) {
    if (USER) {
      const int4 r = static_cast<const int4*>(a.recs)[rbase + sidx];
      if ((uint32_t)r.z - id_lo < (uint32_t)W) {
        const int slot = atomicAdd(s.n, 1);
        s.x[slot] = r.x; s.y[slot] = r.y; s.z[slot] = r.z;
        s.idx[slot] = (unsigned short)r.w;
      }
    } else {
      const int2 oc = static_cast<const int2*>(a.recs)[rbase + sidx];
      const uint32_t b = (uint32_t)(oc.y & 0x7fffffff);
      if (b - id_lo < (uint32_t)W && row_kept((int)((uint32_t)oc.x >> kOccShift), part, parts)) {
        const float g = a.coeff[b];
        const int slot = atomicAdd(s.n, 1);
        s.x[slot] = oc.x & kOccMask;
        s.y[slot] = __float_as_int(oc.y < 0 ? -g : g);
        s.z[slot] = oc.y;
        s.idx[slot] = (unsigned short)((uint32_t)oc.x >> kOccShift);
      }
    }
  }
  __syncthreads();
  const int n_rec = *s.n;
#pragma unroll
  for (int q = 0; q < PT; ++q) {
    const int c = tid + q * kBlock;
    key[q] = -1;
    if (c < n_rec) {
      const int local = s.idx[c];
      key[q] = local | (atomicAdd(&s.cnt[local], 1) << 8);
    }
  }
  ++sub;
  if (sub * W >= tile_ids) { sub = 0; cend = s.pre[wt + 1]; }
  else cend = c0;
  return n_rec;
}

template <class F>
__device__ __forceinline__ void rerank_by_id(const OwnerLds& s, int tid, int n_rec) {
  constexpr int PT = F::PT;
  int at[PT];
  unsigned short ent[PT];
#pragma unroll
  for (int q = 0; q < PT; ++q) {
    const int pos = tid + q * kBlock;
    at[q] = -1;
    if (pos < n_rec) {
      ent[q] = s.idx[pos];
      const int r = F::TAG_SLOT ? (int)s.rowof[ent[q] >> kTagShift] : ent[q] >> kTagShift;
      const uint32_t mine = (uint32_t)s.z[ent[q] & kTagMask];
      const int lo = s.start[r], cnt = s.cnt[r];
      int before = 0;
      for (int j = lo; j < lo + cnt; ++j)
        before += (uint32_t)s.z[s.idx[j] & kTagMask] < mine ? 1 : 0;
      at[q] = lo + before;
    }
  }
  __syncthreads();
#pragma unroll
  for (int q = 0; q < PT; ++q)
    if (at[q] >= 0) s.idx[at[q]] = ent[q];
  __syncthreads();
}

template <class F>
__device__ __forceinline__ bool leave_part_sums(const OwnerArgs& a, const OwnerLds& s, int tid, int k, int part,
                                                int parts, bool finisher, int row_t, const float4& acc, float*& slots,
                                                int& lc) {
  constexpr int D = F::D, R = F::R;
  float* sbase = a.scratch;
  asm volatile("" : "+s"(sbase));
  slots = sbase + (int64_t)split_slot(a.split, a.nb)[k] * (R * D);
  int t3 = tid;
  asm volatile("" : "+v"(t3));
  lc = 4 * (t3 % F::LPR);
  if (finisher) st4(slots + (int64_t)part * (R * D) + row_t * D + lc, acc);
  __threadfence();
  __syncthreads();
  if (tid == 0) {
    *s.last = atomicAdd(split_arrive(a.split, a.nb) + k, 1) == parts - 1;
    if (*s.last) split_arrive(a.split, a.nb)[k] = 0;
  }
  __syncthreads();
  const bool last = *s.last != 0;
  __syncthreads();
  return last;
}

template <class F>
__device__ __forceinline__ float4 sum_part_slots(const float* slots, int lc, int parts, int row_t, bool finisher) {
  constexpr int D = F::D, R = F::R;
  __threadfence();
  float4 acc = zero4();
  if (finisher) {
    for (int q = 0; q < parts; ++q) {
      const float4 p = ld4(slots + (int64_t)q * (R * D) + row_t * D + lc);
      acc.x += p.x; acc.y += p.y; acc.z += p.z; acc.w += p.w;
    }
  }
  return acc;
}

template <int D, bool USER, bool FUSE_ADAM, bool DET, int RPWX = 0>
__global__ __launch_bounds__(kBlock, YR_OWNER_WAVES) void owner_pass_kernel(OwnerArgs a) {
  using F = OwnerForm<D, USER, FUSE_ADAM, DET, RPWX>;
  constexpr int LPR = F::LPR, GPW = F::GPW, RPW = F::RPW, R = F::R, DEAL_BAR = F::DEAL_BAR, CAP = F::CAP, PT = F::PT;
  constexpr bool DEAL = F::DEAL, TAG_SLOT = F::TAG_SLOT, LOOKUP = F::LOOKUP;
  __shared__ int s_pre[kTileGroup + 1];
  __shared__ int s_base[kTileGroup];
  __shared__ int s_cnt[kWave];
  __shared__ int s_start[kWave];
  __shared__ int s_light[kWave + 1];
  __shared__ unsigned char s_slotof[DEAL ? kWave : 1];
  __shared__ unsigned char s_rowof[DEAL ? kWave : 1];
  __shared__ int s_x[CAP];
  __shared__ int s_y[CAP];
  __shared__ int s_z[(USER || DET) ? CAP : 1];
  __shared__ unsigned short s_idx[CAP];
  __shared__ float4 s_own[USER ? R * LPR : 1];
  __shared__ float4 s_heavy[kWavesPerBlock][LPR];
  __shared__ float s_red[kWavesPerBlock];
  __shared__ int s_scan[kWavesPerBlock];
  __shared__ int s_n;
  const int tid = threadIdx.x, lane = tid & (kWave - 1), wave = tid / kWave;
  const int grp = lane / LPR, l = lane % LPR;
  const bool finisher = grp < RPW;
  const int row_l = wave * RPW + (finisher ? grp : 0);
  float loss = 0.0f;
  __shared__ int s_last;
  const OwnerLds s = {s_pre, s_base, s_cnt, s_start, s_rowof, s_x, s_y, s_z, s_idx, s_scan, &s_n, &s_last};
  if (USER && (int)blockIdx.x < a.build_blocks) {
    build_splits(a, blockIdx.x);
    return;
  }
  const int hb = USER ? a.build_blocks : a.helper_blocks;
  const bool helper = !USER && (int)blockIdx.x < hb;
  const int owners = (int)gridDim.x - hb;
#ifdef YR_STAMPS
  bool first_bucket = true;
  int walk_iters = 0, heavy_iters = 0;
#endif
  YR_STAMP(0);

  for (int ks = helper ? (int)blockIdx.x : a.bucket_begin + (int)blockIdx.x - hb;
       helper ? ks == (int)blockIdx.x : ks < a.bucket_end; ks += owners) {
    int k, part = 0, parts = 1;
    int4 cnt = make_int4(0, 0, 0, 0);
    if (!USER && a.split) cnt = *reinterpret_cast<const int4*>(a.split);
    int k_own = ks;
    if (!helper && a.order) k_own = a.order[ks];
    const int c_tasks = __builtin_amdgcn_readfirstlane(cnt.x), c_slots = __builtin_amdgcn_readfirstlane(cnt.y);
    const int c_rows = __builtin_amdgcn_readfirstlane(cnt.z);
    const bool pools_hold = USER || !a.split || (c_tasks <= kMaxTasks && c_slots <= kMaxSlots);
    const int tile_tasks = (USER || !a.split || !pools_hold) ? 0 : c_tasks;
    const bool rows_hold = !USER && YR_ROWSPLIT && a.split && c_rows <= kMaxRowTasks && tile_tasks + c_rows <= kMaxTasks;
    const bool row_helper = YR_ROWSPLIT && helper && ks >= tile_tasks;
    if (row_helper) {
      const int j = kMaxTasks - 1 - ks;
      if (!rows_hold || j >= c_rows) break;
      const int2 task = split_row_tasks(a.split, a.nb)[j];
      k = __builtin_amdgcn_readfirstlane(task.x);
      part = __builtin_amdgcn_readfirstlane(task.y);
      if (k < a.bucket_begin || k >= a.bucket_end) break;
    } else if (helper) {
      if (ks >= tile_tasks) break;
      const int4 task = split_tasks(a.split, a.nb)[ks];
      k = __builtin_amdgcn_readfirstlane(task.x);
      part = __builtin_amdgcn_readfirstlane(task.y);
      if (k < a.bucket_begin || k >= a.bucket_end) break;
    } else {
      k = __builtin_amdgcn_readfirstlane(k_own);
    }
    if (!USER && a.split) {
      const int word = __builtin_amdgcn_readfirstlane(split_parts(a.split)[k]);
      if (word > 1 && pools_hold) parts = word;
      if (YR_ROWSPLIT && word < 0 && rows_hold) parts = word;
    }
    if (row_helper && parts >= 0) break;
    const int t_begin = parts < 0 ? 0 : __builtin_amdgcn_readfirstlane(a.T * part / parts);
    const int t_end = parts < 0 ? a.T : __builtin_amdgcn_readfirstlane(a.T * (part + 1) / parts);
    int row_t = row_l;
    int row_f = k * R + row_t;
    bool valid_f = finisher && row_f < a.rows && (USER || row_kept(row_t, part, parts));
    uint32_t o_f = (uint32_t)(row_f * D + 4 * l);
    bool bound = false;
    if (USER && finisher) s_own[row_l * LPR + l] = valid_f ? ld4o(a.own_old, o_f) : zero4();
    YR_STAMP(1);
    RowSums<LPR, GPW> sums;
    sums.clear();

    for (int tg0 = t_begin; tg0 < t_end; tg0 += kTileGroup) {
      const int nt = min(kTileGroup, t_end - tg0);
      const int total = scan_segments(a, s, tid, k, tg0, nt);
      YR_STAMP(2);

      for (int c0 = 0, cend = 0, sub = 0; c0 < total; c0 = cend) {
        cend = min(total, c0 + CAP);
        int wt = 0;
        bool windowed = false;
        if (DET) windowed = cut_chunk_at_tiles<CAP>(s_pre, nt, c0, total, cend, wt);
        if (tid < kWave) s_cnt[tid] = 0;
        if (DET && tid == 0) s_n = 0;
        __syncthreads();
        int key[PT];
        int n_rec = cend - c0;
        if (DET && windowed) {
          n_rec = load_window<F>(a, s, tid, part, parts, tg0, wt, c0, sub, cend, key);
          if (n_rec == 0) {
            __syncthreads();
            continue;
          }
        } else {
        uint32_t addr[PT];
#pragma unroll
        for (int q = 0; q < PT; ++q) {
          const int j = c0 + tid + q * kBlock;
          key[q] = j < cend ? 0 : -1;
          int tlo = 0, thi = nt;
          while (thi - tlo > 1) {
            const int mid = (tlo + thi) >> 1;
            if (s_pre[mid] <= j) tlo = mid; else thi = mid;
          }
          addr[q] = j < cend ? (uint32_t)(s_base[tlo] + (j - s_pre[tlo])) : 0u;
        }
        if (USER) {
          int4 r[PT];
#pragma unroll
          for (int q = 0; q < PT; ++q)
            r[q] = *reinterpret_cast<const int4*>(static_cast<const char*>(a.recs) + (uint32_t)(addr[q] * 16u));
#pragma unroll
          for (int q = 0; q < PT; ++q)
            if (key[q] >= 0) {
              const int c = tid + q * kBlock;
              s_x[c] = r[q].x; s_y[c] = r[q].y; s_z[c] = r[q].z;
              key[q] = r[q].w | (atomicAdd(&s_cnt[r[q].w], 1) << 8);
            }
        } else {
          int2 oc[PT];
          float g[PT];
#pragma unroll
          for (int q = 0; q < PT; ++q)
            oc[q] = *reinterpret_cast<const int2*>(static_cast<const char*>(a.recs) + (uint32_t)(addr[q] * 8u));
#pragma unroll
          for (int q = 0; q < PT; ++q)
            if (!row_kept((int)((uint32_t)oc[q].x >> kOccShift), part, parts)) key[q] = -1;
#pragma unroll
          for (int q = 0; q < PT; ++q) {
            const uint32_t b = key[q] >= 0 ? (uint32_t)(oc[q].y & 0x7fffffff) : 0u;
            g[q] = *reinterpret_cast<const float*>(reinterpret_cast<const char*>(a.coeff) + (uint32_t)(b * 4u));
          }
#pragma unroll
          for (int q = 0; q < PT; ++q)
            if (key[q] >= 0) {
              const int c = tid + q * kBlock;
              const int local = (int)((uint32_t)oc[q].x >> kOccShift);
              s_x[c] = oc[q].x & kOccMask;
              s_y[c] = __float_as_int(oc[q].y < 0 ? -g[q] : g[q]);
              if (DET) s_z[c] = oc[q].y;
              key[q] = local | (atomicAdd(&s_cnt[local], 1) << 8);
            }
        }
        }
        __syncthreads();
        if (wave == 0) {
          if (DEAL && !bound) {
            int n_deal = n_rec;
            if (!USER && YR_ROWSPLIT && parts < 0) {
              n_deal = s_cnt[lane];
#pragma unroll
              for (int m = 1; m < kWave; m <<= 1) n_deal += __shfl_xor(n_deal, m, kWave);
            }
            if (n_deal >= DEAL_BAR) {
              deal_rows<R, RPW>(s_cnt, s_slotof, s_rowof, lane, a.heavy_t);
            } else {
              s_slotof[lane] = (unsigned char)lane;
              s_rowof[lane] = (unsigned char)lane;
            }
            __builtin_amdgcn_fence(__ATOMIC_ACQ_REL, "wavefront");
            __builtin_amdgcn_wave_barrier();
          }
          const int row = DEAL ? (int)s_rowof[lane] : lane;
          const int c = s_cnt[row];
          const bool heavy = c > a.heavy_t;
          const int cl = heavy ? 0 : c, ch = heavy ? c : 0;
          const int il = wave_inclusive_scan(cl, lane), ih = wave_inclusive_scan(ch, lane);
          const int total_light = __shfl(il, kWave - 1, kWave);
          s_light[lane] = il - cl;
          if (lane == kWave - 1) s_light[kWave] = il;
          if (!USER && YR_ROWSPLIT && lane == kWave - 1) s_n = il + ih;
          s_start[row] = heavy ? total_light + ih - ch : il - cl;
        }
        bound = true;
        __syncthreads();
        if (!USER && YR_ROWSPLIT && parts < 0) n_rec = __builtin_amdgcn_readfirstlane(s_n);
#pragma unroll
        for (int q = 0; q < PT; ++q)
          if (key[q] >= 0) {
            const int row = key[q] & 255;
            const int tag = TAG_SLOT ? (int)s_slotof[row] : row;
            s_idx[s_start[row] + (key[q] >> 8)] = (unsigned short)((tid + q * kBlock) | (tag << kTagShift));
          }
        __syncthreads();
        if (DET) rerank_by_id<F>(s, tid, n_rec);
        {
          float4 cur = zero4();
          walk_stream<D, USER, false, LOOKUP>(a, s_idx, s_x, s_y, s_z, s_own, s_slotof, s_light[wave * RPW],
                                            s_light[wave * RPW + RPW], grp, GPW, wave * RPW, grp, l, sums, cur, loss);
#ifdef YR_STAMPS
          if (first_bucket) walk_iters += walk_steps<USER>(s_light[wave * RPW + RPW] - s_light[wave * RPW], GPW);
#endif
        }
        if (n_rec - s_light[kWave] > 0) {
#pragma unroll 1
          for (int r = 0; r < R; ++r) {
            const int cnt = s_cnt[r];
            if (cnt <= a.heavy_t) continue;
            const int lo = s_start[r];
            float4 t = zero4();
            walk_stream<D, USER, true, LOOKUP>(a, s_idx, s_x, s_y, s_z, s_own, s_slotof, lo, lo + cnt, wave * GPW + grp,
                                             kWavesPerBlock * GPW, 0, grp, l, sums, t, loss);
#ifdef YR_STAMPS
            if (first_bucket) { walk_iters += walk_steps<USER>(cnt, kWavesPerBlock * GPW); heavy_iters += 1; }
#endif
            cross_group_sum<LPR>(t);
            if (grp == 0) s_heavy[wave][l] = t;
            __syncthreads();
            if (finisher && row_l == (DEAL ? (int)s_slotof[r] : r)) {
#pragma unroll
              for (int w = 0; w < kWavesPerBlock; ++w) {
                const float4 h = s_heavy[w][l];
                sums.total.x += h.x; sums.total.y += h.y; sums.total.z += h.z; sums.total.w += h.w;
              }
            }
            __syncthreads();
          }
        }
        __syncthreads();
      }
    }

    YR_STAMP(3);
    float4 acc = sums.finish(grp);
    if (DEAL) {
      if (bound) row_t = s_rowof[row_l];
      row_f = k * R + row_t;
      valid_f = row_f < a.rows && (USER || row_kept(row_t, part, parts));
      int t2 = tid;
      asm volatile("" : "+v"(t2));
      o_f = (uint32_t)(row_f * D + 4 * (t2 % LPR));
    }
    if (!USER && parts > 1) {
      float* slots;
      int lc;
      if (!leave_part_sums<F>(a, s, tid, k, part, parts, finisher, row_t, acc, slots, lc)) continue;
      acc = sum_part_slots<F>(slots, lc, parts, row_t, finisher);
    }
    if (valid_f) {
      if (FUSE_ADAM) {
        float4 own = USER ? s_own[row_t * LPR + l] : ld4o(a.own_old, o_f);
        float4 M = ld4o(a.m, o_f), V = ld4o(a.v, o_f);
        adam_element(own.x, acc.x, M.x, V.x, a.adam.c, a.adam.decoupled);
        adam_element(own.y, acc.y, M.y, V.y, a.adam.c, a.adam.decoupled);
        adam_element(own.z, acc.z, M.z, V.z, a.adam.c, a.adam.decoupled);
        adam_element(own.w, acc.w, M.w, V.w, a.adam.c, a.adam.decoupled);
        st4(a.own_new + o_f, own);
        st4(a.m + o_f, M);
        st4(a.v + o_f, V);
      } else {
        st4(a.grad_out + o_f, acc);
      }
    }
    YR_STAMP(4);
    if (USER) __syncthreads();
    YR_STAMP(5);
#ifdef YR_STAMPS
    if (first_bucket) {
      if (lane == 0) g_walk_iters[(blockIdx.x + (USER ? 0 : 4096)) * 4 + wave] = walk_iters;
      if (tid == 0) {
        g_stamps[(blockIdx.x + (USER ? 0 : 4096)) * 8 + 6] = k;
        g_stamps[(blockIdx.x + (USER ? 0 : 4096)) * 8 + 7] = heavy_iters;
      }
    }
    first_bucket = false;
#endif
  }

  if (USER) {
    const float total = block_sum(loss, s_red);
    if (tid == 0) a.loss_partials[(int)blockIdx.x - hb] = total;
    if ((int)blockIdx.x == hb)
      for (int i = owners + tid; i < YR_LOSS_PARTIALS; i += kBlock) a.loss_partials[i] = 0.0f;
  } else if (a.finalize && (int)blockIdx.x == hb) {
    float s = 0.0f;
    for (int i = tid; i < YR_LOSS_PARTIALS; i += kBlock) s += a.loss_partials[i];
    const float total = block_sum(s, s_red);
    if (tid == 0) {
      const float v = total * a.inv_batch;
      if (a.loss_out) a.loss_out[0] = v;
      if (a.loss_accum) a.loss_accum[0] += (double)v;
    }
  }
}

__global__ __launch_bounds__(kBlock) void pull_loss_finalize_kernel(const float* __restrict__ partials, float scale,
                                                                    float* __restrict__ loss_out,
                                                                    double* __restrict__ loss_accum) {
  __shared__ float s_red[kWavesPerBlock];
  float s = 0.0f;
  for (int i = threadIdx.x; i < YR_LOSS_PARTIALS; i += kBlock) s += partials[i];
  const float total = block_sum(s, s_red);
  if (threadIdx.x == 0) {
    const float v = total * scale;
    if (loss_out) loss_out[0] = v;
    if (loss_accum) loss_accum[0] += (double)v;
  }
}

inline size_t align16(size_t x) { return (x + 15) & ~(size_t)15; }
struct PullPlan {
  int pt, tile, T, shiftU, shiftI, narrow_users, nbU, nbI;
  size_t o_offU, o_offI, o_rec, o_occ, o_coeff, o_split, o_scratch, bytes;
};
inline size_t split_bytes(int nbI) {
  return 16 + (size_t)3 * align16((size_t)nbI * 4) + (size_t)kMaxTasks * sizeof(int4) + (size_t)kMaxRowTasks * sizeof(int2);
}

inline int tile_pt(int64_t B) {
  int pt = 4;
  while (pt > 1 && (B + (int64_t)kPartThreads * pt - 1) / ((int64_t)kPartThreads * pt) < kMinTiles) pt >>= 1;
  return pt;
}

inline PullPlan make_plan(int64_t B, int64_t nU, int64_t nI, int D, bool upper_bound) {
  PullPlan p;
  p.shiftI = bucket_shift(D);
  const int R = 1 << p.shiftI;
  p.narrow_users = (nU + R - 1) / R < kNarrowBelow && R > kNarrowRows;
  p.shiftU = p.narrow_users ? kNarrowShift : p.shiftI;
  p.nbU = (int)((nU + (1 << p.shiftU) - 1) >> p.shiftU);
  p.nbI = (int)((nI + (1 << p.shiftI) - 1) >> p.shiftI);
  p.pt = tile_pt(B);
  p.tile = kPartThreads * p.pt;
  p.T = (int)((B + p.tile - 1) / p.tile);
  const int64_t T = upper_bound ? ((B + 4095) / 4096 > 2 * kMinTiles ? (B + 4095) / 4096 : 2 * kMinTiles) : p.T;
  const int64_t slots = upper_bound ? B + 4096 : (int64_t)p.T * p.tile;
  size_t o = 0;
  p.o_offU = o; o += align16((size_t)T * (p.nbU + 1) * 4);
  p.o_offI = o; o += align16((size_t)T * (p.nbI + 1) * 4);
  p.o_rec = o; o += align16((size_t)slots * sizeof(int4));
  p.o_occ = o; o += align16((size_t)slots * 2 * sizeof(int2));
  p.o_coeff = o; o += align16((size_t)(B > 0 ? B : 1) * 4);
  p.o_split = o; o += align16(split_bytes(p.nbI));
  p.o_scratch = o; o += (size_t)kMaxSlots * 1024 * 4;
  p.bytes = o;
  return p;
}

struct SplitRule {
  int split_min, split_target, row_min, row_target, row_quad, row_max_parts;
};
inline SplitRule split_rule(int64_t B, int nbI, int D) {
  SplitRule r;
  const double avg = 2.0 * (double)B / (double)nbI;
  const int by_avg_min = (int)(YR_SPLIT_AVG_MIN * avg), by_avg_target = (int)(YR_SPLIT_AVG_TARGET * avg);
  r.split_min = by_avg_min > kSplitMin ? by_avg_min : kSplitMin;
  r.split_target = by_avg_target > kSplitTarget ? by_avg_target : kSplitTarget;
  const int row_avg_min = (int)(YR_ROWSPLIT_AVG_MIN * avg), row_avg_target = (int)(YR_ROWSPLIT_AVG_TARGET * avg);
  r.row_min = row_avg_min > kRowSplitMin ? row_avg_min : kRowSplitMin;
  r.row_target = row_avg_target > kRowSplitTarget ? row_avg_target : kRowSplitTarget;
  r.row_max_parts = D == 128 ? 2 : 4;
  r.row_quad = r.row_max_parts >= 4 && r.row_target < 0x7fffffff / 3 ? 3 * r.row_target : 0x7fffffff;
  if (!YR_ROWSPLIT) { r.row_min = 0x7fffffff; r.row_quad = 0x7fffffff; r.row_max_parts = 1; }
  return r;
}

}

using namespace yr;

static int pull_check_common(int64_t B, int D, int64_t num_users, int64_t num_items, const void* workspace,
                             int64_t workspace_bytes) {
  if (B < 0 || num_users <= 0 || num_items <= 0 || B > 0x3fffffff) return YR_ERR_BADARG;
  if (D != 16 && D != 32 && D != 64 && D != 128) return YR_ERR_UNSUPPORTED;
  const PullPlan pl = make_plan(0, num_users, num_items, D, false);
  if (pl.nbU > kMaxBuckets || pl.nbI > kMaxBuckets) return YR_ERR_UNSUPPORTED;
  if (num_users > kOccMask) return YR_ERR_UNSUPPORTED;
  if (!workspace || (reinterpret_cast<uintptr_t>(workspace) & 15u) != 0) return YR_ERR_BADARG;
  if ((int64_t)make_plan(B, num_users, num_items, D, false).bytes > workspace_bytes) return YR_ERR_BADARG;
  return 0;
}

#ifdef YR_STAMPS
extern "C" int yr_debug_read_stamps(long long* host, int n) {
  return (int)hipMemcpyFromSymbol(host, HIP_SYMBOL(g_stamps), sizeof(long long) * n);
}
extern "C" int yr_debug_read_walk_iters(int* host, int n) {
  return (int)hipMemcpyFromSymbol(host, HIP_SYMBOL(g_walk_iters), sizeof(int) * n);
}
#endif

extern "C" int64_t yr_bpr_mf_pull_workspace_bytes(int64_t max_batch, int64_t num_users, int64_t num_items, int D) {
  if (max_batch < 0 || num_users <= 0 || num_items <= 0) return YR_ERR_BADARG;
  if (D != 16 && D != 32 && D != 64 && D != 128) return YR_ERR_UNSUPPORTED;
  return (int64_t)make_plan(max_batch, num_users, num_items, D, true).bytes;
}

extern "C" int yr_bpr_mf_pull_index(const int64_t* user, const int64_t* pos, const int64_t* neg, int64_t B, int D,
                                    int64_t num_users, int64_t num_items, void* workspace, int64_t workspace_bytes,
                                    int32_t* err_flag, void* stream) {
  const int rc = pull_check_common(B, D, num_users, num_items, workspace, workspace_bytes);
  if (rc) return rc;
  if (B == 0) return 0;
  if (!user || !pos || !neg) return YR_ERR_BADARG;
  const PullPlan p = make_plan(B, num_users, num_items, D, false);
  char* w = static_cast<char*>(workspace);
  int32_t* offU = (int32_t*)(w + p.o_offU);
  int32_t* offI = (int32_t*)(w + p.o_offI);
  int4* rec = (int4*)(w + p.o_rec);
  int2* occ = (int2*)(w + p.o_occ);
  const int stage_off = (((p.nbU > p.nbI ? p.nbU : p.nbI) + 1) + 3) & ~3;
  const size_t lds = (size_t)stage_off * 4 + (size_t)p.tile * 16;
  const dim3 grid(p.T, 2);
  hipStream_t s = (hipStream_t)stream;
#define YR_PART_CASE(PT)                                                                                         \
  case PT: {                                                                                                     \
    static bool raised = false;                    \
    if (!raised && lds > 65536) {                                                                                \
      const hipError_t e = hipFuncSetAttribute(reinterpret_cast<const void*>(&tile_partition_kernel<PT>),        \
                                               hipFuncAttributeMaxDynamicSharedMemorySize, 160 * 1024 - 256);    \
      if (e != hipSuccess) return (int)e;                                                                        \
      raised = true;                                                                                             \
    }                                                                                                            \
    hipLaunchKernelGGL((tile_partition_kernel<PT>), grid, dim3(kPartThreads), lds, s, user, pos, neg, B, num_users, \
                       num_items, p.shiftU, p.shiftI, p.nbU, p.nbI, offU, offI, rec, occ, err_flag, stage_off,   \
                       (int32_t*)(w + p.o_split));                                                              \
  } break
  switch (p.pt) {
    YR_PART_CASE(1);
    YR_PART_CASE(2);
    YR_PART_CASE(4);
    default: return YR_ERR_BADARG;
  }
#undef YR_PART_CASE
  return launch_status();
}

template <int D>
static int pull_apply_impl(const float* U_old, float* U_new, float* I, float* mU, float* vU, float* mI, float* vI,
                           float* gradI_out, int64_t B, int64_t nU, int64_t nI, float inv_batch, const PullAdam& adam,
                           int deterministic, void* workspace, float* loss_partials, float* loss_out,
                           double* loss_accum, int phases, int64_t item_begin, int64_t item_end,
                           const int32_t* item_order, hipStream_t s) {
  const PullPlan p = make_plan(B, nU, nI, D, false);
  char* w = static_cast<char*>(workspace);
  const bool want_loss = loss_out || loss_accum;
  if (phases & YR_PULL_USER_PHASE) {
    OwnerArgs ua{};
    ua.own_old = U_old; ua.own_new = U_new; ua.other = I; ua.m = mU; ua.v = vU; ua.grad_out = nullptr;
    ua.off = (const int32_t*)(w + p.o_offU); ua.recs = w + p.o_rec; ua.coeff = (float*)(w + p.o_coeff);
    ua.loss_partials = loss_partials;
    ua.nb = p.nbU; ua.T = p.T; ua.tile_stride = p.tile; ua.rows = (int)nU;
    ua.bucket_begin = 0; ua.bucket_end = p.nbU;
    ua.order = nullptr;
    ua.heavy_t = kHeavyRow; ua.inv_batch = inv_batch; ua.adam = adam;
    ua.build_blocks = (p.nbI * kBuildLanes + kBlock - 1) / kBlock;
    ua.b_off = (const int32_t*)(w + p.o_offI); ua.b_nb = p.nbI;
    const SplitRule rule = split_rule(B, p.nbI, D);
    ua.b_split_min = rule.split_min; ua.b_split_target = rule.split_target;
    ua.b_rowsplit_min = rule.row_min; ua.b_rowsplit_quad = rule.row_quad;
    ua.split = w + p.o_split;
    const int gu = (p.nbU < YR_LOSS_PARTIALS ? p.nbU : YR_LOSS_PARTIALS) + ua.build_blocks;
    if (p.narrow_users && deterministic)
      hipLaunchKernelGGL((owner_pass_kernel<D, true, true, true, 1>), dim3(gu), dim3(kBlock), 0, s, ua);
    else if (p.narrow_users)
      hipLaunchKernelGGL((owner_pass_kernel<D, true, true, false, 1>), dim3(gu), dim3(kBlock), 0, s, ua);
    else if (deterministic)
      hipLaunchKernelGGL((owner_pass_kernel<D, true, true, true>), dim3(gu), dim3(kBlock), 0, s, ua);
    else
      hipLaunchKernelGGL((owner_pass_kernel<D, true, true, false>), dim3(gu), dim3(kBlock), 0, s, ua);
  }
  const bool items = (phases & YR_PULL_ITEM_PHASE) && item_end > item_begin;
  if (items) {
    OwnerArgs ia{};
    ia.own_old = I; ia.own_new = I; ia.other = U_old; ia.m = mI; ia.v = vI; ia.grad_out = gradI_out;
    ia.off = (const int32_t*)(w + p.o_offI); ia.recs = w + p.o_occ; ia.coeff = (float*)(w + p.o_coeff);
    ia.loss_partials = loss_partials; ia.loss_out = loss_out; ia.loss_accum = loss_accum;
    ia.finalize = want_loss ? 1 : 0;
    ia.nb = p.nbI; ia.T = p.T; ia.tile_stride = 2 * p.tile; ia.rows = (int)nI;
    ia.bucket_begin = (int)(item_begin >> p.shiftI);
    ia.bucket_end = (int)((item_end + (1 << p.shiftI) - 1) >> p.shiftI);
    ia.order = (item_order && ia.bucket_begin == 0 && ia.bucket_end == p.nbI) ? item_order : nullptr;
    ia.heavy_t = kHeavyRow; ia.inv_batch = inv_batch; ia.adam = adam;
    ia.helper_blocks = kMaxTasks;
    ia.split = w + p.o_split;
    ia.scratch = (float*)(w + p.o_scratch);
    int gi = ia.bucket_end - ia.bucket_begin;
    if (gi > kMaxOwnerGrid) gi = kMaxOwnerGrid;
    gi += ia.helper_blocks;
    if (gradI_out && deterministic)
      hipLaunchKernelGGL((owner_pass_kernel<D, false, false, true>), dim3(gi), dim3(kBlock), 0, s, ia);
    else if (gradI_out)
      hipLaunchKernelGGL((owner_pass_kernel<D, false, false, false>), dim3(gi), dim3(kBlock), 0, s, ia);
    else if (deterministic)
      hipLaunchKernelGGL((owner_pass_kernel<D, false, true, true>), dim3(gi), dim3(kBlock), 0, s, ia);
    else
      hipLaunchKernelGGL((owner_pass_kernel<D, false, true, false>), dim3(gi), dim3(kBlock), 0, s, ia);
  } else if (want_loss) {
    hipLaunchKernelGGL(pull_loss_finalize_kernel, dim3(1), dim3(kBlock), 0, s, loss_partials, inv_batch, loss_out,
                       loss_accum);
  }
  return launch_status();
}

extern "C" int yr_bpr_mf_pull_item_buckets(int64_t num_items, int D) {
  if (num_items <= 0 || (D != 16 && D != 32 && D != 64 && D != 128)) return YR_ERR_BADARG;
  const int sh = bucket_shift(D);
  return (int)((num_items + (1 << sh) - 1) >> sh);
}

extern "C" int yr_bpr_mf_pull_split_summary(const void* workspace, int64_t workspace_bytes, int64_t B, int D,
                                            int64_t num_users, int64_t num_items, int32_t* counters_out,
                                            int32_t* parts_out, int32_t* rule_out, void* stream) {
  if (!rule_out || B <= 0 || num_users <= 0 || num_items <= 0) return YR_ERR_BADARG;
  if (D != 16 && D != 32 && D != 64 && D != 128) return YR_ERR_UNSUPPORTED;
  const PullPlan p = make_plan(B, num_users, num_items, D, false);
  const SplitRule r = split_rule(B, p.nbI, D);
  const int32_t rule[8] = {r.split_min, r.split_target, r.row_min, r.row_target, r.row_quad, r.row_max_parts,
                           kMaxRowTasks, YR_ROWSPLIT};
  for (int i = 0; i < 8; ++i) rule_out[i] = rule[i];
  if (!workspace) return (counters_out || parts_out) ? YR_ERR_BADARG : 0;
  const int rc = pull_check_common(B, D, num_users, num_items, workspace, workspace_bytes);
  if (rc) return rc;
  const char* blk = static_cast<const char*>(workspace) + p.o_split;
  hipStream_t s = (hipStream_t)stream;
  hipError_t e = hipSuccess;
  if (counters_out) e = hipMemcpyAsync(counters_out, blk, 16, hipMemcpyDeviceToHost, s);
  if (e == hipSuccess && parts_out)
    e = hipMemcpyAsync(parts_out, blk + 16, (size_t)p.nbI * 4, hipMemcpyDeviceToHost, s);
  if (e == hipSuccess) e = hipStreamSynchronize(s);
  return (int)e;
}

extern "C" int yr_bpr_mf_pull_apply_ordered(const float* U_old, float* U_new, float* I, float* mU, float* vU,
                                            float* mI, float* vI, float* gradI_out, int64_t B, int D,
                                            int64_t num_users, int64_t num_items, float inv_batch, double lr,
                                            double step_size, double bc2_sqrt, double beta1, double beta2, double eps,
                                            double weight_decay, int mode, int deterministic, void* workspace,
                                            int64_t workspace_bytes, float* loss_partials, float* loss_out,
                                            double* loss_accum, int phases, int64_t item_row_begin,
                                            int64_t item_row_end, const int32_t* item_bucket_order, void* stream) {
  int rc = pull_check_common(B, D, num_users, num_items, workspace, workspace_bytes);
  if (rc) return rc;
  if (!(phases & (YR_PULL_USER_PHASE | YR_PULL_ITEM_PHASE))) return YR_ERR_BADARG;
  if (item_row_begin < 0 || item_row_end > num_items || item_row_begin > item_row_end) return YR_ERR_BADARG;
  const int R = 1 << bucket_shift(D);
  if (item_row_begin % R != 0 || (item_row_end % R != 0 && item_row_end != num_items)) return YR_ERR_BADARG;
  if (!U_old || !U_new || U_old == U_new || !I || !mU || !vU || !loss_partials) return YR_ERR_BADARG;
  if (!gradI_out && (!mI || !vI)) return YR_ERR_BADARG;
  if (mode != YR_OPT_ADAM && mode != YR_OPT_ADAMW) return YR_ERR_UNSUPPORTED;
  const PullAdam c = {adam_scalars(lr, step_size, bc2_sqrt, beta1, beta2, eps, weight_decay), mode == YR_OPT_ADAMW};
  hipStream_t s = (hipStream_t)stream;
#define YR_APPLY_CASE(DD)                                                                                       \
  case DD:                                                                                                      \
    return pull_apply_impl<DD>(U_old, U_new, I, mU, vU, mI, vI, gradI_out, B, num_users, num_items, inv_batch,  \
                               c, deterministic ? 1 : 0, workspace, loss_partials, loss_out, loss_accum, phases,      \
                               item_row_begin, item_row_end, item_bucket_order, s)
  switch (D) {
    YR_APPLY_CASE(16);
    YR_APPLY_CASE(32);
    YR_APPLY_CASE(64);
    YR_APPLY_CASE(128);
    default: return YR_ERR_UNSUPPORTED;
  }
#undef YR_APPLY_CASE
}

extern "C" int yr_bpr_mf_pull_apply(const float* U_old, float* U_new, float* I, float* mU, float* vU, float* mI,
                                    float* vI, float* gradI_out, int64_t B, int D, int64_t num_users,
                                    int64_t num_items, float inv_batch, double lr, double step_size, double bc2_sqrt,
                                    double beta1, double beta2, double eps, double weight_decay, int mode,
                                    int deterministic, void* workspace, int64_t workspace_bytes,
                                    float* loss_partials, float* loss_out, double* loss_accum, int phases,
                                    int64_t item_row_begin, int64_t item_row_end, void* stream) {
  return yr_bpr_mf_pull_apply_ordered(U_old, U_new, I, mU, vU, mI, vI, gradI_out, B, D, num_users, num_items,
                                      inv_batch, lr, step_size, bc2_sqrt, beta1, beta2, eps, weight_decay, mode,
                                      deterministic, workspace, workspace_bytes, loss_partials, loss_out, loss_accum,
                                      phases, item_row_begin, item_row_end, nullptr, stream);
}

extern "C" int yr_bpr_mf_pull_step(const float* U_old, float* U_new, float* I, float* mU, float* vU, float* mI,
                                   float* vI, float* gradI_out, const int64_t* user, const int64_t* pos,
                                   const int64_t* neg, int64_t B, int D, int64_t num_users, int64_t num_items,
                                   float inv_batch, double lr, double step_size, double bc2_sqrt, double beta1,
                                   double beta2, double eps, double weight_decay, int mode, int deterministic,
                                   void* workspace, int64_t workspace_bytes, float* loss_partials, float* loss_out,
                                   double* loss_accum, int32_t* err_flag, void* stream) {
  if (mode != YR_OPT_ADAM && mode != YR_OPT_ADAMW) return YR_ERR_UNSUPPORTED;
  if (!U_old || !U_new || U_old == U_new || !I || !mU || !vU || !loss_partials) return YR_ERR_BADARG;
  if (!gradI_out && (!mI || !vI)) return YR_ERR_BADARG;
  int rc = yr_bpr_mf_pull_index(user, pos, neg, B, D, num_users, num_items, workspace, workspace_bytes, err_flag,
                                stream);
  if (rc) return rc;
  return yr_bpr_mf_pull_apply(U_old, U_new, I, mU, vU, mI, vI, gradI_out, B, D, num_users, num_items, inv_batch, lr,
                              step_size, bc2_sqrt, beta1, beta2, eps, weight_decay, mode, deterministic, workspace,
                              workspace_bytes, loss_partials, loss_out, loss_accum,
                              YR_PULL_USER_PHASE | YR_PULL_ITEM_PHASE, 0, num_items, stream);
}
```

yelprecommendation_amd/engine.py:

```python
from __future__ import annotations

import torch

from . import _lib
from ._lib import EngineError, check

LOSS_PARTIALS = 2048
FLAG_BAD_USER, FLAG_BAD_ITEM = 1, 2
OPT_ADAM, OPT_ADAMW = 0, 1
PULL_USER_PHASE, PULL_ITEM_PHASE = 1, 2
SUPPORTED_WIDTHS = (16, 32, 64, 128)
WIDE_WIDTHS = (256, 512, 1024)
MF_WIDTHS = SUPPORTED_WIDTHS + WIDE_WIDTHS


_raw_stream = getattr(torch._C, "_cuda_getCurrentRawStream", None)


def _stream() -> int:
    if _raw_stream is not None:
        return _raw_stream(torch.cuda.current_device())
    return torch.cuda.current_stream().cuda_stream


def _dev(t: torch.Tensor, dtype, name: str) -> int:
    if not isinstance(t, torch.Tensor):
        raise EngineError(f"{name}: expected a tensor, got {type(t).__name__}")
    if not t.is_cuda:
        raise EngineError(f"{name}: tensor is on {t.device}; the engine runs on MI355X only (no CPU fallback)")
    if t.dtype != dtype:
        raise EngineError(f"{name}: dtype {t.dtype}, expected {dtype}")
    if not t.is_contiguous():
        raise EngineError(f"{name}: tensor must be contiguous")
    return t.data_ptr()


def _rows(t: torch.Tensor, dtype, name: str) -> int:
    if isinstance(t, torch.Tensor) and t.dim() == 2 and t.is_cuda and t.dtype == dtype and t.stride(1) == 1 \
            and t.stride(0) >= t.shape[1]:
        return t.data_ptr()
    return _dev(t, dtype, name)


def _opt(t, dtype, name):
    return None if t is None else _dev(t, dtype, name)


def _table_dims(U: torch.Tensor, I: torch.Tensor):
    if U.dim() != 2 or I.dim() != 2 or U.shape[1] != I.shape[1]:
        raise EngineError(f"tables must be [rows, D] with equal D, got {tuple(U.shape)} / {tuple(I.shape)}")
    return U.shape[0], I.shape[0], U.shape[1]


def new_error_flag(device) -> torch.Tensor:
    return torch.zeros(1, dtype=torch.int32, device=device)


def raise_on_flag(flag: torch.Tensor, what: str = "index"):
    v = int(flag.item())
    if v:
        kinds = [k for b, k in ((FLAG_BAD_USER, "user"), (FLAG_BAD_ITEM, "item")) if v & b]
        flag.zero_()
        raise IndexError(f"{what}: out-of-range {' and '.join(kinds)} id(s) in a batch")


def mf_score(U, I, user, item, out=None, err_flag=None):
    lib = _lib.load()
    nu, ni, d = _table_dims(U, I)
    B = user.numel()
    if item.numel() != B:
        raise EngineError("user and item index tensors differ in length")
    if out is None:
        out = torch.empty(B, dtype=torch.float32, device=U.device)
    check(lib.yr_mf_score(_dev(U, torch.float32, "U"), _dev(I, torch.float32, "I"),
                          _dev(user, torch.int64, "user"), _dev(item, torch.int64, "item"),
                          B, d, nu, ni, _dev(out, torch.float32, "out"),
                          _opt(err_flag, torch.int32, "err_flag"), _stream()), "yr_mf_score")
    return out


def mf_score_backward(U, I, user, item, gout, gradU, gradI, err_flag=None):
    lib = _lib.load()
    nu, ni, d = _table_dims(U, I)
    B = user.numel()
    check(lib.yr_mf_score_backward(_dev(U, torch.float32, "U"), _dev(I, torch.float32, "I"),
                                   _dev(user, torch.int64, "user"), _dev(item, torch.int64, "item"),
                                   _dev(gout, torch.float32, "gout"), B, d, nu, ni,
                                   _dev(gradU, torch.float32, "gradU"), _dev(gradI, torch.float32, "gradI"),
                                   _opt(err_flag, torch.int32, "err_flag"), _stream()), "yr_mf_score_backward")


def bpr_mf_fwd_bwd(U, I, user, pos, neg, gradU, gradI, loss_partials, inv_batch=None, err_flag=None):
    lib = _lib.load()
    nu, ni, d = _table_dims(U, I)
    B = user.numel()
    if pos.numel() != B or neg.numel() != B:
        raise EngineError("user/pos/neg index tensors differ in length")
    if loss_partials.numel() != LOSS_PARTIALS:
        raise EngineError(f"loss_partials must hold {LOSS_PARTIALS} floats")
    if inv_batch is None:
        inv_batch = 1.0 / B if B else 0.0
    if gradU is not None and (gradU.shape != U.shape or gradI.shape != I.shape):
        raise EngineError("gradient buffers must match the table shapes")
    check(lib.yr_bpr_mf_fwd_bwd(_dev(U, torch.float32, "U"), _dev(I, torch.float32, "I"),
                                _dev(user, torch.int64, "user"), _dev(pos, torch.int64, "pos"),
                                _dev(neg, torch.int64, "neg"), B, d, nu, ni, float(inv_batch),
                                _opt(gradU, torch.float32, "gradU"), _opt(gradI, torch.float32, "gradI"),
                                _dev(loss_partials, torch.float32, "loss_partials"),
                                _opt(err_flag, torch.int32, "err_flag"), _stream()), "yr_bpr_mf_fwd_bwd")


PULL_MAX_BUCKETS = 16383
PULL_MAX_USERS = (1 << 26) - 1


def pull_bucket_rows(d):
    return 1024 // int(d)


def pull_supported(num_users, num_items, d):
    if d not in SUPPORTED_WIDTHS:
        return False
    r = pull_bucket_rows(d)
    ru = 4 if (-(-num_users // r) < 768 and r > 4) else r
    return (-(-num_users // ru) <= PULL_MAX_BUCKETS and -(-num_items // r) <= PULL_MAX_BUCKETS
            and num_users <= PULL_MAX_USERS)


def bpr_mf_pull_workspace(max_batch, num_users, num_items, d, device):
    lib = _lib.load()
    n = lib.yr_bpr_mf_pull_workspace_bytes(int(max_batch), int(num_users), int(num_items), int(d))
    if n < 0:
        check(int(n), "yr_bpr_mf_pull_workspace_bytes")
    return torch.empty(int(n), dtype=torch.uint8, device=device)


PULL_RULE_FIELDS = ("split_min", "split_target", "row_min", "row_target", "row_quad", "row_max_parts",
                    "row_task_pool", "row_split_compiled")


def bpr_mf_pull_split_summary(batch, num_users, num_items, d, workspace=None):
    import ctypes
    import numpy as np
    lib = _lib.load()
    rule = (ctypes.c_int32 * 8)()
    counters = (ctypes.c_int32 * 4)()
    nb = int(lib.yr_bpr_mf_pull_item_buckets(int(num_items), int(d)))
    if nb < 0:
        check(nb, "yr_bpr_mf_pull_item_buckets")
    parts = np.zeros(nb, np.int32)
    if workspace is None:
        rc = lib.yr_bpr_mf_pull_split_summary(None, 0, int(batch), int(d), int(num_users), int(num_items), None, None,
                                              rule, None)
    else:
        rc = lib.yr_bpr_mf_pull_split_summary(workspace.data_ptr(), workspace.numel(), int(batch), int(d),
                                              int(num_users), int(num_items), counters, parts.ctypes.data, rule,
                                              _stream())
    check(rc, "yr_bpr_mf_pull_split_summary")
    out = dict(zip(PULL_RULE_FIELDS, (int(v) for v in rule)))
    if workspace is not None:
        out.update(tasks=int(counters[0]), slots=int(counters[1]), row_tasks=int(counters[2]), parts=parts)
    return out


def bpr_mf_pull_step(U_old, U_new, I, mU, vU, mI, vI, user, pos, neg, step, lr, loss_partials, workspace,
                     beta1=0.9, beta2=0.999, eps=1e-8, weight_decay=0.0, decoupled=False, inv_batch=None,
                     gradI_out=None, err_flag=None, loss_out=None, loss_accum=None, deterministic=False):
    lib = _lib.load()
    nu, ni, d = _table_dims(U_old, I)
    B = user.numel()
    if pos.numel() != B or neg.numel() != B:
        raise EngineError("user/pos/neg index tensors differ in length")
    if U_new.shape != U_old.shape or U_new.data_ptr() == U_old.data_ptr():
        raise EngineError("U_new must be a distinct buffer of U_old's shape")
    if loss_partials.numel() != LOSS_PARTIALS:
        raise EngineError(f"loss_partials must hold {LOSS_PARTIALS} floats")
    if inv_batch is None:
        inv_batch = 1.0 / B if B else 0.0
    step_size, bc2_sqrt = adam_scalars(step, lr, beta1, beta2)
    f32 = torch.float32
    check(lib.yr_bpr_mf_pull_step(
        _dev(U_old, f32, "U_old"), _dev(U_new, f32, "U_new"), _dev(I, f32, "I"),
        _dev(mU, f32, "mU"), _dev(vU, f32, "vU"), _opt(mI, f32, "mI"), _opt(vI, f32, "vI"),
        _opt(gradI_out, f32, "gradI_out"),
        _dev(user, torch.int64, "user"), _dev(pos, torch.int64, "pos"), _dev(neg, torch.int64, "neg"),
        B, d, nu, ni, float(inv_batch), float(lr), float(step_size), float(bc2_sqrt), float(beta1), float(beta2),
        float(eps), float(weight_decay), OPT_ADAMW if decoupled else OPT_ADAM, 1 if deterministic else 0,
        _dev(workspace, torch.uint8, "workspace"), workspace.numel(),
        _dev(loss_partials, f32, "loss_partials"), _opt(loss_out, f32, "loss_out"),
        _opt(loss_accum, torch.float64, "loss_accum"), _opt(err_flag, torch.int32, "err_flag"), _stream()),
        "yr_bpr_mf_pull_step")


def triplet_sample(row_user, row_item, avoid_ptr, avoid_idx, num_users, num_items, seed, epoch, shuffle=True,
                   first=0, count=None, err_flag=None):
    lib = _lib.load()
    n_rows = row_user.numel()
    count = n_rows - first if count is None else int(count)
    i64 = torch.int64
    out = [torch.empty(count, dtype=i64, device=row_user.device) for _ in range(3)]
    if avoid_ptr.numel() != num_users + 1:
        raise EngineError("avoid_ptr must hold num_users + 1 offsets")
    check(lib.yr_triplet_sample(_dev(row_user, i64, "row_user"), _dev(row_item, i64, "row_item"), n_rows,
                                _dev(avoid_ptr, i64, "avoid_ptr"),
                                _dev(avoid_idx, i64, "avoid_idx") if avoid_idx.numel() else _dev(avoid_ptr, i64, "avoid_ptr"),
                                int(num_users), int(num_items), int(seed) & (2**64 - 1), int(epoch) & (2**64 - 1),
                                1 if shuffle else 0, int(first), count,
                                *(_dev(t, i64, "out") if count else None for t in out),
                                _opt(err_flag, torch.int32, "err_flag"), _stream()), "yr_triplet_sample")
    return tuple(out)


SPMM_FORM = "rows"


def spmm_csr(graph, X, out=None, accumulate=False, form=None):
    lib = _lib.load()
    n, d = X.shape
    if n != graph.n:
        raise EngineError(f"X has {n} rows, the graph {graph.n}")
    if out is None:
        if accumulate:
            raise EngineError("accumulate needs an output buffer")
        out = torch.empty_like(X)
    form = form or SPMM_FORM
    if form not in ("rows", "sliced"):
        raise EngineError("form must be 'rows' or 'sliced'")
    if form == "sliced":
        check(lib.yr_spmm_csr_sliced(_dev(graph.rowptr, torch.int32, "rowptr"), _dev(graph.col, torch.int32, "col"),
                                     _dev(graph.val, torch.float32, "val"), _dev(X, torch.float32, "X"),
                                     _dev(out, torch.float32, "Y"), n, d, 1 if accumulate else 0,
                                     _opt(graph.row_order, torch.int32, "row_order"), _stream()), "yr_spmm_csr_sliced")
        return out
    check(lib.yr_spmm_csr(_dev(graph.rowptr, torch.int32, "rowptr"), _dev(graph.col, torch.int32, "col"),
                          _dev(graph.val, torch.float32, "val"), _dev(X, torch.float32, "X"),
                          _dev(out, torch.float32, "Y"), n, d, 1 if accumulate else 0,
                          _opt(graph.heavy_rows, torch.int32, "heavy_rows"), graph.n_heavy, graph.heavy_threshold,
                          _stream()), "yr_spmm_csr")
    return out


NGCF_MAX_LAYERS = 8


def _ptr_array(tensors, what):
    import ctypes
    if not 0 < len(tensors) <= NGCF_MAX_LAYERS:
        raise EngineError(f"{what}: between 1 and {NGCF_MAX_LAYERS} layer buffers")
    return (ctypes.c_void_p * len(tensors))(*[_dev(t, torch.float32, what) for t in tensors])


class NGCFRowSet:
    __slots__ = ("flags", "rows", "count", "max_rows", "push")

    def __init__(self, n, device, max_rows, push=False):
        self.flags = torch.empty(n, dtype=torch.int32, device=device)
        self.rows = torch.empty(n, dtype=torch.int32, device=device)
        self.count = torch.empty(1, dtype=torch.int32, device=device)
        self.max_rows, self.push = int(min(max_rows, n)), bool(push)


def ngcf_frontier_mark(num_users, num_items, user_id, pos_ids, neg_ids=None, max_rows=None, push=False):
    lib = _lib.load()
    i64 = torch.int64
    B = user_id.numel()
    out = NGCFRowSet(num_users + num_items, user_id.device, (2 if neg_ids is None else 3) * B if max_rows is None else max_rows, push)
    check(lib.yr_ngcf_frontier_mark(_dev(user_id, i64, "user_id") if B else None, _dev(pos_ids, i64, "pos_ids") if B else None,
                                    _dev(neg_ids, i64, "neg_ids") if (neg_ids is not None and B) else None, B,
                                    num_users, num_items, out.flags.data_ptr(), out.rows.data_ptr(), out.count.data_ptr(),
                                    1, _stream()), "yr_ngcf_frontier_mark")
    return out


def ngcf_frontier_expand(graph, rows, max_rows=None, push=False):
    lib = _lib.load()
    out = NGCFRowSet(graph.n, rows.flags.device, graph.n if max_rows is None else max_rows, push)
    check(lib.yr_ngcf_frontier_expand(_dev(graph.rowptr, torch.int32, "rowptr"), _dev(graph.col, torch.int32, "col"),
                                      graph.n, rows.rows.data_ptr(), rows.count.data_ptr(), rows.max_rows,
                                      out.flags.data_ptr(), out.rows.data_ptr(), out.count.data_ptr(), 1, _stream()),
          "yr_ngcf_frontier_expand")
    return out


def spmm_csr_subset(graph, X, out, row_active=None, accumulate=False, rows=None):
    if rows is not None:
        row_active = rows.flags
    lib = _lib.load()
    n, d = X.shape
    if n != graph.n or out.shape != X.shape:
        raise EngineError(f"X / out must be [{graph.n}, D]")
    check(lib.yr_spmm_csr_subset(_dev(graph.rowptr, torch.int32, "rowptr"), _dev(graph.col, torch.int32, "col"),
                                 _dev(graph.val, torch.float32, "val"), _dev(X, torch.float32, "X"),
                                 _dev(out, torch.float32, "Y"), n, d, 1 if accumulate else 0,
                                 _opt(graph.heavy_rows, torch.int32, "heavy_rows"), graph.n_heavy, graph.heavy_threshold,
                                 _opt(row_active, torch.int32, "row_active"),
                                 None if rows is None else rows.rows.data_ptr(),
                                 None if rows is None else rows.count.data_ptr(), 0 if rows is None else rows.max_rows,
                                 _stream()),
          "yr_spmm_csr_subset")
    return out


def spmm_csr_push_rows(graph, X, out, rows):
    lib = _lib.load()
    n, d = X.shape
    if n != graph.n or out.shape != X.shape:
        raise EngineError(f"X / out must be [{graph.n}, D]")
    check(lib.yr_spmm_csr_push_rows(_dev(graph.rowptr, torch.int32, "rowptr"), _dev(graph.col, torch.int32, "col"),
                                    _dev(graph.val, torch.float32, "val"), _dev(X, torch.float32, "X"),
                                    _dev(out, torch.float32, "Y"), n, d, rows.rows.data_ptr(), rows.count.data_ptr(),
                                    rows.max_rows, _stream()), "yr_spmm_csr_push_rows")
    return out


def ngcf_score(layers, num_users, user_id, pos_ids, neg_ids=None, err_flag=None):
    lib = _lib.load()
    n, d = layers[0].shape
    B = user_id.numel()
    i64 = torch.int64
    pos = torch.empty(B, dtype=torch.float32, device=layers[0].device)
    neg = torch.empty_like(pos) if neg_ids is not None else None
    check(lib.yr_ngcf_score_fwd(_ptr_array(layers, "layers"), len(layers), _dev(user_id, i64, "user_id"),
                                _dev(pos_ids, i64, "pos_ids"), _dev(neg_ids, i64, "neg_ids") if neg_ids is not None else None,
                                B, d, num_users, n - num_users, pos.data_ptr(),
                                neg.data_ptr() if neg is not None else None,
                                err_flag.data_ptr() if err_flag is not None else None, _stream()), "yr_ngcf_score_fwd")
    return pos if neg is None else (pos, neg)


def ngcf_score_backward(layers, dlayers, num_users, user_id, pos_ids, neg_ids, gpos, gneg, err_flag=None):
    lib = _lib.load()
    n, d = layers[0].shape
    i64, f32 = torch.int64, torch.float32
    if len(layers) != len(dlayers):
        raise EngineError("layers / dlayers length mismatch")
    check(lib.yr_ngcf_score_bwd(_ptr_array(layers, "layers"), _ptr_array(dlayers, "dlayers"), len(layers),
                                _dev(user_id, i64, "user_id"), _dev(pos_ids, i64, "pos_ids"),
                                _dev(neg_ids, i64, "neg_ids") if neg_ids is not None else None,
                                _dev(gpos, f32, "gpos"), _dev(gneg, f32, "gneg") if neg_ids is not None else None,
                                user_id.numel(), d, num_users, n - num_users,
                                err_flag.data_ptr() if err_flag is not None else None, _stream()), "yr_ngcf_score_bwd")


def ngcf_dense_fwd(E, Z, W1, W2, out=None, rows=None):
    lib = _lib.load()
    n, d = E.shape
    if out is None:
        out = torch.empty_like(E)
    f32 = torch.float32
    if rows is not None:
        check(lib.yr_ngcf_dense_fwd_rows(_dev(E, f32, "E"), _dev(Z, f32, "Z"), _dev(W1, f32, "W1"), _dev(W2, f32, "W2"),
                                         n, d, _dev(out, f32, "Eout"), rows.rows.data_ptr(), rows.count.data_ptr(),
                                         rows.max_rows, None, _stream()), "yr_ngcf_dense_fwd_rows")
        return out
    check(lib.yr_ngcf_dense_fwd(_dev(E, f32, "E"), _dev(Z, f32, "Z"), _dev(W1, f32, "W1"), _dev(W2, f32, "W2"),
                                n, d, _dev(out, f32, "Eout"), _stream()), "yr_ngcf_dense_fwd")
    return out


def ngcf_dense_bwd(dEout, Eout, E, Z, W1, W2, dE, dW1, dW2, dZ=None, W1T=None, W2T=None, rows=None):
    lib = _lib.load()
    n, d = E.shape
    f32 = torch.float32
    if dZ is None:
        dZ = torch.empty_like(E)
    if W1T is None:
        W1T, W2T = W1.t().contiguous(), W2.t().contiguous()
    if rows is not None:
        r, c, m = rows.rows.data_ptr(), rows.count.data_ptr(), rows.max_rows
        check(lib.yr_ngcf_dense_bwd_weight_rows(_dev(dEout, f32, "dEout"), _dev(Eout, f32, "Eout"), _dev(E, f32, "E"),
                                                _dev(Z, f32, "Z"), n, d, _dev(dW1, f32, "dW1"), _dev(dW2, f32, "dW2"),
                                                r, c, m, _stream()), "yr_ngcf_dense_bwd_weight_rows")
        check(lib.yr_ngcf_dense_bwd_data_rows(_dev(dEout, f32, "dEout"), _dev(Eout, f32, "Eout"), _dev(E, f32, "E"),
                                              _dev(Z, f32, "Z"), _dev(W1T, f32, "W1T"), _dev(W2T, f32, "W2T"), n, d,
                                              _dev(dZ, f32, "dZ"), _dev(dE, f32, "dE"), r, c, m, _stream()),
              "yr_ngcf_dense_bwd_data_rows")
        return dZ
    check(lib.yr_ngcf_dense_bwd_weight(_dev(dEout, f32, "dEout"), _dev(Eout, f32, "Eout"), _dev(E, f32, "E"),
                                       _dev(Z, f32, "Z"), n, d, _dev(dW1, f32, "dW1"), _dev(dW2, f32, "dW2"),
                                       _stream()), "yr_ngcf_dense_bwd_weight")
    check(lib.yr_ngcf_dense_bwd_data(_dev(dEout, f32, "dEout"), _dev(Eout, f32, "Eout"), _dev(E, f32, "E"),
                                     _dev(Z, f32, "Z"), _dev(W1T, f32, "W1T"), _dev(W2T, f32, "W2T"), n, d,
                                     _dev(dZ, f32, "dZ"), _dev(dE, f32, "dE"), _stream()), "yr_ngcf_dense_bwd_data")
    return dZ


ACT_IDENTITY, ACT_SIGMOID, ACT_RELU = 0, 1, 2
COUNT_WORDS, COUNT_SLOTS = 2048, 64


def gemm_f32(A, B, transA=False, transB=False, out=None, bias=None, act=ACT_IDENTITY, accumulate=False,
             split_k=1, alpha_count=None, rowsum=None):
    lib = _lib.load()
    f32 = torch.float32
    M, K = (A.shape[1], A.shape[0]) if transA else (A.shape[0], A.shape[1])
    K2, N = (B.shape[1], B.shape[0]) if transB else (B.shape[0], B.shape[1])
    if K != K2:
        raise EngineError(f"inner dimensions differ: {K} vs {K2}")
    if out is None:
        if accumulate:
            raise EngineError("accumulate needs an output buffer")
        out = (torch.zeros if split_k > 1 else torch.empty)((M, N), dtype=f32, device=A.device)
    if out.shape != (M, N) or out.stride(1) != 1:
        raise EngineError("bad output buffer")
    if alpha_count is not None and alpha_count.numel() != COUNT_WORDS:
        raise EngineError(f"alpha_count: a spread count of {COUNT_WORDS} int32 words")
    if alpha_count is not None or rowsum is not None:
        if rowsum is not None and rowsum.numel() != M:
            raise EngineError("rowsum needs one element per row of op(A)")
        check(lib.yr_gemm_f32_ex(1 if transA else 0, 1 if transB else 0, M, N, K, _rows(A, f32, "A"), A.stride(0),
                                 _rows(B, f32, "B"), B.stride(0), out.data_ptr(), out.stride(0),
                                 _opt(bias, f32, "bias"), int(act), 1 if accumulate else 0, int(split_k),
                                 _opt(alpha_count, torch.int32, "alpha_count"), _opt(rowsum, f32, "rowsum"),
                                 _stream()), "yr_gemm_f32_ex")
        return out
    check(lib.yr_gemm_f32(1 if transA else 0, 1 if transB else 0, M, N, K, _rows(A, f32, "A"), A.stride(0),
                          _rows(B, f32, "B"), B.stride(0), out.data_ptr(), out.stride(0),
                          _opt(bias, f32, "bias"), int(act), 1 if accumulate else 0, int(split_k), _stream()),
          "yr_gemm_f32")
    return out


def spread_count(value, device):
    c = torch.zeros(COUNT_WORDS, dtype=torch.int32, device=device)
    c[0] = int(value)
    return c


def cdae_decode_loss_partials(B, I):
    return int(_lib.load().yr_cdae_decode_loss_partials(int(B), int(I)))


def cdae_decode_loss(z, Wo, bo, target, negative_mask, act, G, partial_loss, count, pred=None):
    lib = _lib.load()
    f32 = torch.float32
    B, H = z.shape
    I = Wo.shape[0]
    if partial_loss.numel() < cdae_decode_loss_partials(B, I) or G.shape != (B, I) or target.shape != (B, I):
        raise EngineError("bad buffers for cdae_decode_loss")
    if count.numel() != COUNT_WORDS:
        raise EngineError(f"count: a spread count of {COUNT_WORDS} int32 words")
    if pred is not None and (pred.shape != G.shape or pred.stride() != G.stride()):
        raise EngineError("pred must have the layout of G")
    check(lib.yr_cdae_decode_loss(_dev(z, f32, "z"), _dev(Wo, f32, "Wo"), _opt(bo, f32, "bo"),
                                  _dev(target, f32, "target"), _opt(negative_mask, f32, "negative_mask"), B, I, H,
                                  int(act), _rows(G, f32, "G"), G.stride(0),
                                  None if pred is None else _rows(pred, f32, "pred"),
                                  _dev(partial_loss, f32, "partial_loss"), _dev(count, torch.int32, "count"),
                                  _stream()), "yr_cdae_decode_loss")
    return G


class TrainLists:
    _pool = {}

    def __init__(self, ptr, idx, users, num_users, num_items, neg_times, neg_seed, drop_seed, p, err_flag=None,
                 extra=None, pool=None, batch_rows=None, targets=None):
        lib = _lib.load()
        B, I = users.numel(), int(num_items)
        dev = users.device
        key = (dev, B, I)
        pool = TrainLists._pool if pool is None else pool
        slot = pool.get(key)
        if slot is None:
            n, parts = B * SPARSE_PARTS * sparse_part_columns(I), B * SPARSE_PARTS
# ... 1075 lines not shown
```

Baseline: 5.052 billion triplets/s.

## Replace item-phase helper blocks with a cost-sorted snake work list

The last split-builder block now builds a device-side work list of item buckets and their split parts. Entries are bucketed by estimated record cost, ordered heaviest first, and laid out in a boustrophedon pattern across a fixed grid width. The item owner pass walks this list with a stride equal to the grid width, replacing the old split between owner and helper blocks and the optional host-computed item order. This aims to balance load across blocks and drop the host-side bincount/argsort; the cost is an extra last-block-arrives histogram and scan on the critical path before the item phase can start.

```diff
diff --git a/include/yelprec_engine.h b/include/yelprec_engine.h
--- a/include/yelprec_engine.h
+++ b/include/yelprec_engine.h
@@ -89,6 +89,11 @@
                          int phases, int64_t item_row_begin, int64_t item_row_end,
                          void *stream);
 int yr_bpr_mf_pull_item_buckets(int64_t num_items, int D);
+int yr_bpr_mf_pull_work_list(const void *workspace, int64_t workspace_bytes, int64_t B, int D,
+                             int64_t num_users, int64_t num_items, int32_t *head_out, int32_t *list_out,
+                             int64_t list_capacity, void *stream);
+int yr_bpr_mf_pull_list_width_override(int width);
+int yr_bpr_mf_pull_list_rule(int rank, int W, int records, int parts, int32_t *out);
 int yr_bpr_mf_pull_split_summary(const void *workspace, int64_t workspace_bytes, int64_t B, int D,
                                  int64_t num_users, int64_t num_items, int32_t *counters_out,
                                  int32_t *parts_out, int32_t *rule_out, void *stream);
diff --git a/yelprecommendation_amd/_lib.py b/yelprecommendation_amd/_lib.py
--- a/yelprecommendation_amd/_lib.py
+++ b/yelprecommendation_amd/_lib.py
@@ -73,6 +73,9 @@
                              _d, _d, _d, _d, _d, _d, _d, _int, _int, _p, _i64, _p, _p, _p, _int, _i64, _i64, _p, _p],
     "yr_bpr_mf_pull_item_buckets": [_i64, _int],
     "yr_bpr_mf_pull_split_summary": [_p, _i64, _i64, _int, _i64, _i64, _p, _p, _p, _p],
+    "yr_bpr_mf_pull_work_list": [_p, _i64, _i64, _int, _i64, _i64, _p, _p, _i64, _p],
+    "yr_bpr_mf_pull_list_width_override": [_int],
+    "yr_bpr_mf_pull_list_rule": [_int, _int, _int, _int, _p],
     "yr_loss_finalize": [_p, _f, _p, _p, _p],
     "yr_mf_scores_gemm": [_p, _p, _p, _i64, _int, _i64, _i64, _p, _i64, _p, _p],
     "yr_mf_eval_topk_planes_bytes": [_i64, _int],
diff --git a/yelprecommendation_amd/bpr_step.py b/yelprecommendation_amd/bpr_step.py
--- a/yelprecommendation_amd/bpr_step.py
+++ b/yelprecommendation_amd/bpr_step.py
@@ -167,17 +167,9 @@
         load = w.view(nb, per).sum(1)
         self._item_order = torch.argsort(load, descending=True, stable=True).to(torch.int32).contiguous()
 
-    def _auto_item_order(self, p, n):
-        rows = self.I.shape[0]
-        ids = torch.cat([p, n])
-        ids = ids[(ids >= 0) & (ids < rows)]
-        self.set_item_order(torch.bincount(ids, minlength=rows)[:rows])
-
     def _step_pull(self, u, p, n, record, global_batch, next_batch=None):
         B = u.numel()
         D = self.U.shape[1]
-        if self._item_order is None and self.auto_item_order and B >= 4 * self.I.shape[0]:
-            self._auto_item_order(p, n)
         inv = 1.0 / global_batch if global_batch else 0.0
         self.t += 1
         multi = self.world_size > 1 or self.split_item_update
@@ -198,15 +190,13 @@
             if with_loss is None:
                 with_loss = bool(phases & engine.PULL_USER_PHASE)
             step_size, bc2_sqrt = engine.adam_scalars(self.t, self.lr, self.betas[0], self.betas[1])
-            order = self._item_order
-            rc = self._lib.yr_bpr_mf_pull_apply_ordered(
+            rc =self._lib.yr_bpr_mf_pull_apply_ordered(
                 self.U.data_ptr(), self._U_alt.data_ptr(), self._pI, self._pmU, self._pvU, self._pmI, self._pvI,
                 self.gI.data_ptr() if multi else None, B, D, self.U.shape[0], rows, inv, self.lr,
                 step_size, bc2_sqrt, self.betas[0], self.betas[1], self.eps, self.wd,
                 engine.OPT_ADAMW if self.decoupled else engine.OPT_ADAM, 1 if self.deterministic else 0,
                 ws.data_ptr(), ws.numel(), self._ppartials, ploss if with_loss else None,
-                paccum if with_loss else None, phases, r0, r1, order.data_ptr() if order is not None else None,
-                engine._stream())
+                paccum if with_loss else None, phases, r0, r1, None, engine._stream())
             if rc:
                 engine.check(rc, "yr_bpr_mf_pull_apply_ordered")
 
diff --git a/yelprecommendation_amd/csrc/bpr_pull.hip b/yelprecommendation_amd/csrc/bpr_pull.hip
--- a/yelprecommendation_amd/csrc/bpr_pull.hip
+++ b/yelprecommendation_amd/csrc/bpr_pull.hip
@@ -1,5 +1,6 @@
 #include "adam.h"
 #include "common.h"
+#include "pull_worklist.h"
 
 namespace yr {
 
@@ -102,21 +103,35 @@
 
 inline int bucket_shift(int D) { return D == 16 ? 6 : D == 32 ? 5 : D == 64 ? 4 : 3; }
 
+__host__ __device__ __forceinline__ size_t split_per(int nbI) { return ((size_t)nbI * 4 + 15) & ~(size_t)15; }
+__device__ __forceinline__ int32_t* split_counters(char* b) { return (int32_t*)b; }
+__device__ __forceinline__ int32_t* split_parts(char* b) { return (int32_t*)(b + 16); }
+__device__ __forceinline__ int32_t* split_slot(char* b, int nbI) { return (int32_t*)(b + 16 + split_per(nbI)); }
+__device__ __forceinline__ int32_t* split_arrive(char* b, int nbI) { return (int32_t*)(b + 16 + 2 * split_per(nbI)); }
+__device__ __forceinline__ int32_t* split_total(char* b, int nbI) { return (int32_t*)(b + 16 + 3 * split_per(nbI)); }
+__host__ __device__ __forceinline__ size_t split_list_offset(int nbI) { return 16 + 4 * split_per(nbI); }
+__device__ __forceinline__ int32_t* split_list(char* b, int nbI) { return (int32_t*)(b + split_list_offset(nbI)); }
+constexpr int kListHead = 4;
+
 template <int PT>
 __global__ __launch_bounds__(kPartThreads) void tile_partition_kernel(
     const int64_t* __restrict__ user, const int64_t* __restrict__ pos, const int64_t* __restrict__ neg, int64_t B,
     int64_t nU, int64_t nI, int shiftU, int shiftI, int nbU, int nbI, int32_t* __restrict__ offU,
     int32_t* __restrict__ offI,
     int4* __restrict__ rec, int2* __restrict__ occ, int32_t* __restrict__ err_flag, int stage_off,
-    int32_t* __restrict__ split_counters) {
+    int32_t* __restrict__ split_block, int list_w) {
   extern __shared__ int32_t s_cnt[];
   __shared__ int s_wave[kPartThreads / kWave];
   int4* s_stage = reinterpret_cast<int4*>(s_cnt + stage_off);
   constexpr int TILE = kPartThreads * PT;
   const int side = blockIdx.y, tile = blockIdx.x, tid = threadIdx.x;
   if (side == 0 && tile == 0) {
-    if (tid < 3) split_counters[tid] = 0;
-    for (int i = tid; i < nbI; i += kPartThreads) split_counters[4 + i] = 1;
+    if (tid < 4) split_block[tid] = 0;
+    for (int i = tid; i < nbI; i += kPartThreads) split_block[4 + i] = 1;
+    int32_t* list = split_list(reinterpret_cast<char*>(split_block), nbI);
+    if (tid < kListHead) list[tid] = tid == 0 ? nbI : tid == 1 ? list_w : 0;
+    const int np = list_positions(nbI, list_w);
+    for (int i = tid; i < np; i += kPartThreads) list[kListHead + i] = i < nbI ? list_entry(i, 0, 1) : kListEnd;
   }
   const int nb = side ? nbI : nbU;
   const int shift = side ? shiftI : shiftU;
@@ -211,8 +226,10 @@
 __device__ long long g_stamps[8192 * 8];
 __device__ int g_walk_iters[8192 * 4];
 #define YR_STAMP(i) do { if (threadIdx.x == 0 && first_bucket) g_stamps[(blockIdx.x + (USER ? 0 : 4096)) * 8 + (i)] = wall_clock64(); } while (0)
+#define YR_STAMP_END(i) do { if (threadIdx.x == 0) g_stamps[(blockIdx.x + (USER ? 0 : 4096)) * 8 + (i)] = wall_clock64(); } while (0)
 #else
 #define YR_STAMP(i)
+#define YR_STAMP_END(i)
 #endif
 
 struct OwnerArgs {
@@ -232,25 +249,17 @@
   int nb, T, tile_stride;
   int rows;
   int bucket_begin, bucket_end;
-  const int32_t* order;
+  const int32_t* list;
   int heavy_t;
   float inv_batch;
   PullAdam adam;
   char* split;
   float* scratch;
   const int32_t* b_off;
-  int helper_blocks, build_blocks, b_nb;
+  int list_w, build_blocks, b_nb;
   int b_split_min, b_split_target;
   int b_rowsplit_min, b_rowsplit_quad;
 };
-
-__host__ __device__ __forceinline__ size_t split_per(int nbI) { return ((size_t)nbI * 4 + 15) & ~(size_t)15; }
-__device__ __forceinline__ int32_t* split_counters(char* b) { return (int32_t*)b; }
-__device__ __forceinline__ int32_t* split_parts(char* b) { return (int32_t*)(b + 16); }
-__device__ __forceinline__ int32_t* split_slot(char* b, int nbI) { return (int32_t*)(b + 16 + split_per(nbI)); }
-__device__ __forceinline__ int32_t* split_arrive(char* b, int nbI) { return (int32_t*)(b + 16 + 2 * split_per(nbI)); }
-__device__ __forceinline__ int4* split_tasks(char* b, int nbI) { return (int4*)(b + 16 + 3 * split_per(nbI)); }
-__device__ __forceinline__ int2* split_row_tasks(char* b, int nbI) { return (int2*)(split_tasks(b, nbI) + kMaxTasks); }
 
 __device__ __forceinline__ void build_splits(const OwnerArgs& a, int builder) {
   const int k = (builder * kBlock + (int)threadIdx.x) / kBuildLanes, j = threadIdx.x % kBuildLanes;
@@ -283,23 +292,19 @@
   if (parts > 1) {
     slot = atomicAdd(split_counters(a.split) + 1, parts);
     const int first = atomicAdd(split_counters(a.split), parts - 1);
-    const bool fits = slot + parts <= kMaxSlots && first + parts - 1 <= kMaxTasks;
-    for (int q = 1; q < parts; ++q)
-      if (first + q - 1 < kMaxTasks) split_tasks(a.split, a.b_nb)[first + q - 1] = make_int4(fits ? k : -1, q, 0, 0);
-    if (!fits) parts = 1;
+    if (slot + parts > kMaxSlots || first + parts - 1 > kMaxTasks) parts = 1;
   }
 #if YR_ROWSPLIT
   else if (total < a.b_split_min && total >= a.b_rowsplit_min) {
     const int S = total >= a.b_rowsplit_quad ? 4 : 2;
-    const int first = atomicAdd(split_counters(a.split) + 2, S - 1);
-    for (int q = 1; q < S; ++q)
-      if (first + q - 1 < kMaxRowTasks) split_row_tasks(a.split, a.b_nb)[first + q - 1] = make_int2(k, q);
+    atomicAdd(split_counters(a.split) + 2, S - 1);
     parts = -S;
   }
 #endif
   split_parts(a.split)[k] = parts;
   split_slot(a.split, a.b_nb)[k] = slot;
   split_arrive(a.split, a.b_nb)[k] = 0;
+  split_total(a.split, a.b_nb)[k] = total;
 }
 
 template <int LPR>
@@ -313,13 +318,85 @@
   }
 }
 
+template <bool REBUILD = false>
 __device__ __forceinline__ int wave_inclusive_scan(int x, int lane) {
+  if (REBUILD) {
+    int self = lane & (kWave - 1);
+    asm volatile("" : "+v"(self));
+#pragma unroll
+    for (int d = 1; d < kWave; d <<= 1) {
+      const int t = __builtin_amdgcn_ds_bpermute((self - d) << 2, x);
+      if (self >= d) x += t;
+    }
+    return x;
+  }
 #pragma unroll
   for (int d = 1; d < kWave; d <<= 1) {
     const int t = __shfl_up(x, d, kWave);
     if (lane >= d) x += t;
   }
   return x;
+}
+
+__device__ __forceinline__ int ld_device(const int32_t* p) {
+  return __hip_atomic_load(p, __ATOMIC_RELAXED, __HIP_MEMORY_SCOPE_AGENT);
+}
+
+__device__ __forceinline__ int parts_in_force(int word, int c_tasks, int c_slots, int c_rows) {
+  const bool pools_hold = c_tasks <= kMaxTasks && c_slots <= kMaxSlots;
+  const int tile_tasks = pools_hold ? c_tasks : 0;
+  const bool rows_hold = YR_ROWSPLIT && c_rows <= kMaxRowTasks && tile_tasks + c_rows <= kMaxTasks;
+  if (word > 1) return pools_hold ? word : 1;
+  if (word < 0) return rows_hold ? word : 1;
+  return 1;
+}
+
+__device__ __forceinline__ void build_work_list(const OwnerArgs& a, int* s_hist, int* s_flag) {
+  const int tid = threadIdx.x, W = a.list_w;
+  __threadfence();
+  __syncthreads();
+  if (tid == 0) {
+    *s_flag = atomicAdd(split_counters(a.split) + 3, 1) == a.build_blocks - 1;
+    if (*s_flag) split_counters(a.split)[3] = 0;
+  }
+  __syncthreads();
+  if (!*s_flag) return;
+  __threadfence();
+  const int32_t* cnt = split_counters(a.split);
+  const int c_tasks = ld_device(cnt), c_slots = ld_device(cnt + 1), c_rows = ld_device(cnt + 2);
+  const int32_t* words = split_parts(a.split);
+  const int32_t* totals = split_total(a.split, a.b_nb);
+  int32_t* list = split_list(a.split, a.b_nb);
+  for (int i = tid; i <= kListClasses; i += kBlock) s_hist[i] = 0;
+  __syncthreads();
+  for (int k = tid; k < a.b_nb; k += kBlock) {
+    const int parts = parts_in_force(ld_device(words + k), c_tasks, c_slots, c_rows);
+    atomicAdd(&s_hist[list_weight_class(list_cost(ld_device(totals + k), parts))], parts < 0 ? -parts : parts);
+  }
+  __syncthreads();
+  if (tid < kWave) {
+    constexpr int PER = kListClasses / kWave;
+    int c[PER], sum = 0;
+#pragma unroll
+    for (int q = 0; q < PER; ++q) { c[q] = s_hist[kListClasses - 1 - (tid * PER + q)]; sum += c[q]; }
+    const int inc = wave_inclusive_scan(sum, tid);
+    int before = inc - sum;
+#pragma unroll
+    for (int q = 0; q < PER; ++q) { s_hist[kListClasses - 1 - (tid * PER + q)] = before; before += c[q]; }
+    if (tid == kWave - 1) s_hist[kListClasses] = inc;
+  }
+  __syncthreads();
+  const int n = s_hist[kListClasses];
+  for (int k = tid; k < a.b_nb; k += kBlock) {
+    const int parts = parts_in_force(ld_device(words + k), c_tasks, c_slots, c_rows);
+    const int np = parts < 0 ? -parts : parts;
+    const int r0 = atomicAdd(&s_hist[list_weight_class(list_cost(ld_device(totals + k), parts))], np);
+    for (int q = 0; q < np; ++q) list[kListHead + list_position(r0 + q, W)] = list_entry(k, q, parts);
+  }
+  const int full = (n + W - 1) / W * W;
+  for (int r = n + tid; r < full; r += kBlock) list[kListHead + list_position(r, W)] = kListEnd;
+  for (int i = full + tid; i < full + W; i += kBlock) list[kListHead + i] = kListEnd;
+  if (tid == 0) { list[0] = n; list[1] = W; }
 }
 
 template <int LPR, int GPW>
@@ -485,6 +562,7 @@
   return tlo;
 }
 
+template <bool REBUILD>
 __device__ __forceinline__ int scan_segments(const OwnerArgs& a, const OwnerLds& s, int tid, int k, int tg0,
                                              int nt) {
   const int lane = tid & (kWave - 1), wave = tid / kWave;
@@ -497,12 +575,12 @@
   }
   int inc = 0, before = 0;
   if (nt > kWave) {
-    inc = wave_inclusive_scan(len, lane);
+    inc = wave_inclusive_scan<REBUILD>(len, lane);
     if (lane == kWave - 1) s.scan[wave] = inc;
     __syncthreads();
     for (int w = 0; w < wave; ++w) before += s.scan[w];
   } else if (wave == 0) {
-    inc = wave_inclusive_scan(len, lane);
+    inc = wave_inclusive_scan<REBUILD>(len, lane);
   }
   if (nt > kWave || wave == 0) {
     s.pre[tid] = before + inc - len;
@@ -667,10 +745,10 @@
   const OwnerLds s = {s_pre, s_base, s_cnt, s_start, s_rowof, s_x, s_y, s_z, s_idx, s_scan, &s_n, &s_last};
   if (USER && (int)blockIdx.x < a.build_blocks) {
     build_splits(a, blockIdx.x);
+    build_work_list(a, s_x, &s_last);
     return;
   }
-  const int hb = USER ? a.build_blocks : a.helper_blocks;
-  const bool helper = !USER && (int)blockIdx.x < hb;
+  const int hb = USER ? a.build_blocks : 0;
   const int owners = (int)gridDim.x - hb;
 #ifdef YR_STAMPS
   bool first_bucket = true;
@@ -678,41 +756,17 @@
 #endif
   YR_STAMP(0);
 
-  for (int ks = helper ? (int)blockIdx.x : a.bucket_begin + (int)blockIdx.x - hb;
-       helper ? ks == (int)blockIdx.x : ks < a.bucket_end; ks += owners) {
-    int k, part = 0, parts = 1;
-    int4 cnt = make_int4(0, 0, 0, 0);
-    if (!USER && a.split) cnt = *reinterpret_cast<const int4*>(a.split);
-    int k_own = ks;
-    if (!helper && a.order) k_own = a.order[ks];
-    const int c_tasks = __builtin_amdgcn_readfirstlane(cnt.x), c_slots = __builtin_amdgcn_readfirstlane(cnt.y);
-    const int c_rows = __builtin_amdgcn_readfirstlane(cnt.z);
-    const bool pools_hold = USER || !a.split || (c_tasks <= kMaxTasks && c_slots <= kMaxSlots);
-    const int tile_tasks = (USER || !a.split || !pools_hold) ? 0 : c_tasks;
-    const bool rows_hold = !USER && YR_ROWSPLIT && a.split && c_rows <= kMaxRowTasks && tile_tasks + c_rows <= kMaxTasks;
-    const bool row_helper = YR_ROWSPLIT && helper && ks >= tile_tasks;
-    if (row_helper) {
-      const int j = kMaxTasks - 1 - ks;
-      if (!rows_hold || j >= c_rows) break;
-      const int2 task = split_row_tasks(a.split, a.nb)[j];
-      k = __builtin_amdgcn_readfirstlane(task.x);
-      part = __builtin_amdgcn_readfirstlane(task.y);
-      if (k < a.bucket_begin || k >= a.bucket_end) break;
-    } else if (helper) {
-      if (ks >= tile_tasks) break;
-      const int4 task = split_tasks(a.split, a.nb)[ks];
-      k = __builtin_amdgcn_readfirstlane(task.x);
-      part = __builtin_amdgcn_readfirstlane(task.y);
-      if (k < a.bucket_begin || k >= a.bucket_end) break;
-    } else {
-      k = __builtin_amdgcn_readfirstlane(k_own);
-    }
-    if (!USER && a.split) {
-      const int word = __builtin_amdgcn_readfirstlane(split_parts(a.split)[k]);
-      if (word > 1 && pools_hold) parts = word;
-      if (YR_ROWSPLIT && word < 0 && rows_hold) parts = word;
-    }
-    if (row_helper && parts >= 0) break;
+  for (int ks = USER ? a.bucket_begin + (int)blockIdx.x - hb : (int)blockIdx.x; USER ? ks < a.bucket_end : ks < a.b_nb;
+       ks += USER ? owners : a.list_w) {
+    int k = ks, part = 0, parts = 1;
+    if (!USER) {
+      const int e = __builtin_amdgcn_readfirstlane(a.list[ks]);
+      if (e < 0) break;
+      k = list_bucket(e);
+      part = list_part(e);
+      parts = list_parts(e);
+      if (k < a.bucket_begin || k >= a.bucket_end) continue;
+    }
     const int t_begin = parts < 0 ? 0 : __builtin_amdgcn_readfirstlane(a.T * part / parts);
     const int t_end = parts < 0 ? a.T : __builtin_amdgcn_readfirstlane(a.T * (part + 1) / parts);
     int row_t = row_l;
@@ -727,7 +781,7 @@
 
     for (int tg0 = t_begin; tg0 < t_end; tg0 += kTileGroup) {
       const int nt = min(kTileGroup, t_end - tg0);
-      const int total = scan_segments(a, s, tid, k, tg0, nt);
+      const int total = scan_segments<!USER>(a, s, tid, k, tg0, nt);
       YR_STAMP(2);
 
       for (int c0 = 0, cend = 0, sub = 0; c0 < total; c0 = cend) {
@@ -819,7 +873,7 @@
           const int c = s_cnt[row];
           const bool heavy = c > a.heavy_t;
           const int cl = heavy ? 0 : c, ch = heavy ? c : 0;
-          const int il = wave_inclusive_scan(cl, lane), ih = wave_inclusive_scan(ch, lane);
+          const int il = wave_inclusive_scan<!USER>(cl, lane), ih = wave_inclusive_scan<!USER>(ch, lane);
           const int total_light = __shfl(il, kWave - 1, kWave);
           s_light[lane] = il - cl;
           if (lane == kWave - 1) s_light[kWave] = il;
@@ -908,7 +962,7 @@
     }
     YR_STAMP(4);
     if (USER) __syncthreads();
-    YR_STAMP(5);
+    YR_STAMP_END(5);
 #ifdef YR_STAMPS
     if (first_bucket) {
       if (lane == 0) g_walk_iters[(blockIdx.x + (USER ? 0 : 4096)) * 4 + wave] = walk_iters;
@@ -957,8 +1011,9 @@
   int pt, tile, T, shiftU, shiftI, narrow_users, nbU, nbI;
   size_t o_offU, o_offI, o_rec, o_occ, o_coeff, o_split, o_scratch, bytes;
 };
+inline int list_capacity(int nbI) { return nbI + kMaxTasks + kMaxRowTasks + 2 * kMaxOwnerGrid; }
 inline size_t split_bytes(int nbI) {
-  return 16 + (size_t)3 * align16((size_t)nbI * 4) + (size_t)kMaxTasks * sizeof(int4) + (size_t)kMaxRowTasks * sizeof(int2);
+  return split_list_offset(nbI) + (size_t)(kListHead + list_capacity(nbI)) * 4;
 }
 
 inline int tile_pt(int64_t B) {
@@ -1014,6 +1069,49 @@
 
 using namespace yr;
 
+static int g_list_width_override = 0;
+template <int D>
+static int resident_item_workgroups(int* w_out) {
+  static int cached[16] = {0};
+  int dev = 0;
+  hipError_t e = hipGetDevice(&dev);
+  if (e != hipSuccess) return (int)e;
+  const int slot = dev >= 0 && dev < 16 ? dev : 0;
+  if (!cached[slot] || dev != slot) {
+    int per_cu = 0x7fffffff, n = 0, cus = 0;
+    const void* forms[4] = {reinterpret_cast<const void*>(&owner_pass_kernel<D, false, false, false>),
+                            reinterpret_cast<const void*>(&owner_pass_kernel<D, false, false, true>),
+                            reinterpret_cast<const void*>(&owner_pass_kernel<D, false, true, false>),
+                            reinterpret_cast<const void*>(&owner_pass_kernel<D, false, true, true>)};
+    for (const void* f : forms) {
+      e = hipOccupancyMaxActiveBlocksPerMultiprocessor(&n, f, kBlock, 0);
+      if (e != hipSuccess) return (int)e;
+      per_cu = n < per_cu ? n : per_cu;
+    }
+    e = hipDeviceGetAttribute(&cus, hipDeviceAttributeMultiprocessorCount, dev);
+    if (e != hipSuccess) return (int)e;
+    int w = per_cu * cus;
+    w = w < 1 ? 1 : w > kMaxOwnerGrid ? kMaxOwnerGrid : w;
+    if (dev != slot) { *w_out = w; return 0; }
+    cached[slot] = w;
+  }
+  *w_out = cached[slot];
+  return 0;
+}
+static int list_width(int D, int* w_out) {
+  if (g_list_width_override > 0) {
+    *w_out = g_list_width_override < kMaxOwnerGrid ? g_list_width_override : kMaxOwnerGrid;
+    return 0;
+  }
+  switch (D) {
+    case 16: return resident_item_workgroups<16>(w_out);
+    case 32: return resident_item_workgroups<32>(w_out);
+    case 64: return resident_item_workgroups<64>(w_out);
+    case 128: return resident_item_workgroups<128>(w_out);
+    default: return YR_ERR_UNSUPPORTED;
+  }
+}
+
 static int pull_check_common(int64_t B, int D, int64_t num_users, int64_t num_items, const void* workspace,
                              int64_t workspace_bytes) {
   if (B < 0 || num_users <= 0 || num_items <= 0 || B > 0x3fffffff) return YR_ERR_BADARG;
@@ -1058,6 +1156,8 @@
   const size_t lds = (size_t)stage_off * 4 + (size_t)p.tile * 16;
   const dim3 grid(p.T, 2);
   hipStream_t s = (hipStream_t)stream;
+  int list_w = 0;
+  if (const int e = list_width(D, &list_w)) return e;
 #define YR_PART_CASE(PT)                                                                                         \
   case PT: {                                                                                                     \
     static bool raised = false;                    \
@@ -1069,7 +1169,7 @@
     }                                                                                                            \
     hipLaunchKernelGGL((tile_partition_kernel<PT>), grid, dim3(kPartThreads), lds, s, user, pos, neg, B, num_users, \
                        num_items, p.shiftU, p.shiftI, p.nbU, p.nbI, offU, offI, rec, occ, err_flag, stage_off,   \
-                       (int32_t*)(w + p.o_split));                                                              \
+                       (int32_t*)(w + p.o_split), list_w);                                                      \
   } break
   switch (p.pt) {
     YR_PART_CASE(1);
@@ -1086,9 +1186,11 @@
                            float* gradI_out, int64_t B, int64_t nU, int64_t nI, float inv_batch, const PullAdam& adam,
                            int deterministic, void* workspace, float* loss_partials, float* loss_out,
                            double* loss_accum, int phases, int64_t item_begin, int64_t item_end,
-                           const int32_t* item_order, hipStream_t s) {
+                           hipStream_t s) {
   const PullPlan p = make_plan(B, nU, nI, D, false);
   char* w = static_cast<char*>(workspace);
+  int list_w = 0;
+  if (const int e = list_width(D, &list_w)) return e;
   const bool want_loss = loss_out || loss_accum;
   if (phases & YR_PULL_USER_PHASE) {
     OwnerArgs ua{};
@@ -1097,7 +1199,7 @@
     ua.loss_partials = loss_partials;
     ua.nb = p.nbU; ua.T = p.T; ua.tile_stride = p.tile; ua.rows = (int)nU;
     ua.bucket_begin = 0; ua.bucket_end = p.nbU;
-    ua.order = nullptr;
+    ua.list = nullptr; ua.list_w = list_w;
     ua.heavy_t = kHeavyRow; ua.inv_batch = inv_batch; ua.adam = adam;
     ua.build_blocks = (p.nbI * kBuildLanes + kBlock - 1) / kBlock;
     ua.b_off = (const int32_t*)(w + p.o_offI); ua.b_nb = p.nbI;
@@ -1125,14 +1227,12 @@
     ia.nb = p.nbI; ia.T = p.T; ia.tile_stride = 2 * p.tile; ia.rows = (int)nI;
     ia.bucket_begin = (int)(item_begin >> p.shiftI);
     ia.bucket_end = (int)((item_end + (1 << p.shiftI) - 1) >> p.shiftI);
-    ia.order = (item_order && ia.bucket_begin == 0 && ia.bucket_end == p.nbI) ? item_order : nullptr;
+    ia.list = (const int32_t*)(w + p.o_split + split_list_offset(p.nbI)) + kListHead; ia.list_w = list_w;
+    ia.b_nb = list_capacity(p.nbI);
     ia.heavy_t = kHeavyRow; ia.inv_batch = inv_batch; ia.adam = adam;
-    ia.helper_blocks = kMaxTasks;
     ia.split = w + p.o_split;
     ia.scratch = (float*)(w + p.o_scratch);
-    int gi = ia.bucket_end - ia.bucket_begin;
-    if (gi > kMaxOwnerGrid) gi = kMaxOwnerGrid;
-    gi += ia.helper_blocks;
+    const int gi = list_w < p.nbI + kMaxTasks ? list_w : p.nbI + kMaxTasks;
     if (gradI_out && deterministic)
       hipLaunchKernelGGL((owner_pass_kernel<D, false, false, true>), dim3(gi), dim3(kBlock), 0, s, ia);
     else if (gradI_out)
@@ -1177,6 +1277,46 @@
   return (int)e;
 }
 
+extern "C" int yr_bpr_mf_pull_work_list(const void* workspace, int64_t workspace_bytes, int64_t B, int D,
+                                        int64_t num_users, int64_t num_items, int32_t* head_out, int32_t* list_out,
+                                        int64_t list_capacity_out, void* stream) {
+  if (!head_out || B <= 0) return YR_ERR_BADARG;
+  const int rc = pull_check_common(B, D, num_users, num_items, workspace, workspace_bytes);
+  if (rc) return rc;
+  int w_now = 0;
+  if (const int e = list_width(D, &w_now)) return e;
+  const PullPlan p = make_plan(B, num_users, num_items, D, false);
+  const char* blk = static_cast<const char*>(workspace) + p.o_split + split_list_offset(p.nbI);
+  hipStream_t s = (hipStream_t)stream;
+  int32_t head[kListHead];
+  hipError_t e = hipMemcpyAsync(head, blk, sizeof(head), hipMemcpyDeviceToHost, s);
+  if (e == hipSuccess) e = hipStreamSynchronize(s);
+  if (e != hipSuccess) return (int)e;
+  const int n = head[0], w = head[1];
+  if (n < 1 || w < 1 || w > kMaxOwnerGrid || n > list_capacity(p.nbI) - 2 * w) return YR_ERR_BADARG;
+  const int positions = list_positions(n, w);
+  head_out[0] = n; head_out[1] = w; head_out[2] = positions; head_out[3] = w_now;
+  if (!list_out) return 0;
+  if (list_capacity_out < positions) return YR_ERR_BADARG;
+  e = hipMemcpyAsync(list_out, blk + kListHead * 4, (size_t)positions * 4, hipMemcpyDeviceToHost, s);
+  if (e == hipSuccess) e = hipStreamSynchronize(s);
+  return (int)e;
+}
+
+extern "C" int yr_bpr_mf_pull_list_width_override(int width) {
+  if (width < 0) return YR_ERR_BADARG;
+  g_list_width_override = width;
+  return 0;
+}
+
+extern "C" int yr_bpr_mf_pull_list_rule(int rank, int W, int records, int parts, int32_t* out) {
+  if (!out || rank < 0 || W < 1 || records < 0) return YR_ERR_BADARG;
+  const int pos = list_position(rank, W), cost = list_cost(records, parts);
+  out[0] = pos; out[1] = pos % W; out[2] = pos / W; out[3] = cost; out[4] = list_weight_class(cost);
+  out[5] = list_positions(rank, W);
+  return 0;
+}
+
 extern "C" int yr_bpr_mf_pull_apply_ordered(const float* U_old, float* U_new, float* I, float* mU, float* vU,
                                             float* mI, float* vI, float* gradI_out, int64_t B, int D,
                                             int64_t num_users, int64_t num_items, float inv_batch, double lr,
@@ -1185,6 +1325,7 @@
                                             int64_t workspace_bytes, float* loss_partials, float* loss_out,
                                             double* loss_accum, int phases, int64_t item_row_begin,
                                             int64_t item_row_end, const int32_t* item_bucket_order, void* stream) {
+  (void)item_bucket_order;
   int rc = pull_check_common(B, D, num_users, num_items, workspace, workspace_bytes);
   if (rc) return rc;
   if (!(phases & (YR_PULL_USER_PHASE | YR_PULL_ITEM_PHASE))) return YR_ERR_BADARG;
@@ -1200,7 +1341,7 @@
   case DD:                                                                                                      \
     return pull_apply_impl<DD>(U_old, U_new, I, mU, vU, mI, vI, gradI_out, B, num_users, num_items, inv_batch,  \
                                c, deterministic ? 1 : 0, workspace, loss_partials, loss_out, loss_accum, phases,      \
-                               item_row_begin, item_row_end, item_bucket_order, s)
+                               item_row_begin, item_row_end, s)
   switch (D) {
     YR_APPLY_CASE(16);
     YR_APPLY_CASE(32);
diff --git a/yelprecommendation_amd/csrc/pull_worklist.h b/yelprecommendation_amd/csrc/pull_worklist.h
--- /dev/null
+++ b/yelprecommendation_amd/csrc/pull_worklist.h
@@ -0,0 +1,44 @@
+#pragma once
+
+#if defined(__HIPCC__)
+#define YR_LIST_FN __host__ __device__ __forceinline__
+#else
+#define YR_LIST_FN inline
+#endif
+
+namespace yr {
+
+constexpr int kListBucketBits = 14, kListPartBits = 6, kListPartsBits = 7;
+constexpr int kListEnd = -1;
+
+YR_LIST_FN int list_entry(int bucket, int part, int parts) {
+  int code = 0;
+  for (int s = -parts; s > 1; s >>= 1) ++code;
+  return bucket | (part << kListBucketBits) | ((parts > 0 ? parts : 1) << (kListBucketBits + kListPartBits)) |
+         (code << (kListBucketBits + kListPartBits + kListPartsBits));
+}
+YR_LIST_FN int list_bucket(int e) { return e & ((1 << kListBucketBits) - 1); }
+YR_LIST_FN int list_part(int e) { return (e >> kListBucketBits) & ((1 << kListPartBits) - 1); }
+YR_LIST_FN int list_parts(int e) {
+  const int code = (e >> (kListBucketBits + kListPartBits + kListPartsBits)) & 3;
+  return code ? -(1 << code) : (e >> (kListBucketBits + kListPartBits)) & ((1 << kListPartsBits) - 1);
+}
+
+YR_LIST_FN int list_position(int rank, int W) {
+  const int trip = rank / W, i = rank - trip * W;
+  return trip * W + ((trip & 1) ? W - 1 - i : i);
+}
+YR_LIST_FN int list_positions(int n, int W) { return ((n + W - 1) / W + 1) * W; }
+
+YR_LIST_FN int list_cost(int records, int parts) {
+  if (parts > 1) return (records + parts - 1) / parts;
+  if (parts < 0) return (records + (-parts) - 1) / (-parts) + (records - records / (-parts)) / 4;
+  return records;
+}
+constexpr int kListClasses = 256, kListClassShift = 3;
+YR_LIST_FN int list_weight_class(int cost) {
+  const int c = cost >> kListClassShift;
+  return c < kListClasses - 1 ? c : kListClasses - 1;
+}
+
+}
diff --git a/yelprecommendation_amd/engine.py b/yelprecommendation_amd/engine.py
--- a/yelprecommendation_amd/engine.py
+++ b/yelprecommendation_amd/engine.py
@@ -161,6 +161,27 @@
     if workspace is not None:
         out.update(tasks=int(counters[0]), slots=int(counters[1]), row_tasks=int(counters[2]), parts=parts)
     return out
+
+
+def bpr_mf_pull_work_list(batch, num_users, num_items, d, workspace):
+    import ctypes
+    import numpy as np
+    lib = _lib.load()
+    head = (ctypes.c_int32 * 4)()
+    args = (workspace.data_ptr(), workspace.numel(), int(batch), int(d), int(num_users), int(num_items))
+    check(lib.yr_bpr_mf_pull_work_list(*args, head, None, 0, _stream()), "yr_bpr_mf_pull_work_list")
+    raw = np.zeros(int(head[2]), np.int32)
+    check(lib.yr_bpr_mf_pull_work_list(*args, head, raw.ctypes.data, raw.size, _stream()), "yr_bpr_mf_pull_work_list")
+    end = raw < 0
+    code = (raw >> 27) & 3
+    return dict(items=int(head[0]), width=int(head[1]), width_now=int(head[3]),
+                bucket=np.where(end, -1, raw & 0x3fff).astype(np.int32),
+                part=np.where(end, 0, (raw >> 14) & 63).astype(np.int32),
+                parts=np.where(end, 0, np.where(code > 0, -(1 << code), (raw >> 20) & 127)).astype(np.int32))
+
+
+def pull_list_width_override(width):
+    check(_lib.load().yr_bpr_mf_pull_list_width_override(int(width)), "yr_bpr_mf_pull_list_width_override")
 
 
 def bpr_mf_pull_step(U_old, U_new, I, mU, vU, mI, vI, user, pos, neg, step, lr, loss_partials, workspace,
```

After: 4.867 billion triplets/s. 3.7% lower.
